# second-state/qwen3_asr_rs

Hardware: AMD Instinct MI355X
Metric: audio-seconds/sec (RTFx) Qwen3-ASR-0.6B greedy, 30s clips (higher is better)
Workload: dtype bf16; 1 GPU; Qwen3-ASR-0.6b bf16, batch=1 x 30s synthetic 16kHz clip per GPU, 100 new tokens (fixed, EOS ignored); clips_per_gpu=1, parallelism=dp1 (independent utterances per GPU, no data-path collective)

## Files before the change

qwen3_asr_rs_amd/csrc/engine.cpp:

```cpp
#include <hip/hip_runtime.h>

#include <sched.h>

#include <chrono>
#include <cmath>
#include <cstdio>
#include <cstring>
#include <map>
#include <memory>
#include <mutex>
#include <thread>

#include "engine_internal.h"

using namespace q3a;

namespace {

thread_local std::string g_last_error;

constexpr int kGemvMaxSeq = 2;

template <typename T>
void upload(DevBuf& b, const std::vector<T>& v, hipStream_t s) {
  b.ensure(std::max<size_t>(v.size() * sizeof(T), 16));
  if (!v.empty()) HIPCHK(hipMemcpyAsync(b.p, v.data(), v.size() * sizeof(T), hipMemcpyHostToDevice, s));
}

struct ProfEvent {
  int kclass;
  double bytes;
  hipEvent_t a, b;
};

template <class Build>
std::pair<std::vector<int32_t>, std::vector<int32_t>> concat_prompts(int B, Build&& build) {
  std::vector<int32_t> ids, lens(B);
  for (int s = 0; s < B; ++s) {
    lens[s] = build(s, nullptr);
    const size_t o = ids.size();
    ids.resize(o + lens[s]);
    build(s, ids.data() + o);
  }
  return {std::move(ids), std::move(lens)};
}

void require_utterance_ptrs(const char* what, const float* const* ptrs, int B) {
  for (int u = 0; u < B; ++u)
    if (!ptrs[u]) fail(std::string(what) + ": null utterance pointer");
}

}

namespace q3a {
struct KnobEntry { const char* key; const char* env; std::atomic<int> Knobs::*field; };
static const KnobEntry kKnobTable[] = {
    {"gemm256_min_tiles", "Q3A_GEMM256_MIN_TILES", &Knobs::gemm256_min_tiles},
    {"gemm256_persist", "Q3A_GEMM256_PERSIST", &Knobs::gemm256_persist},
    {"gemm256_group_m", "Q3A_GEMM256_GROUP_M", &Knobs::gemm256_group_m},
    {"dattn_batched_min_wgs", "Q3A_DATTN_BATCHED_MIN_WGS", &Knobs::dattn_batched_min_wgs},
    {"decode_group_size", "Q3A_DECODE_GROUP", &Knobs::decode_group_size},
    {"decode_parallel_groups", "Q3A_DECODE_PARALLEL", &Knobs::decode_parallel_groups},
    {"fuse_qkrope", "Q3A_FUSE_QKROPE", &Knobs::fuse_qkrope},
    {"skinny_q", "Q3A_SKINNY_Q", &Knobs::skinny_q},
    {"eos_run_ahead", "Q3A_EOS_RUN_AHEAD", &Knobs::eos_run_ahead},
    {"skinny_glu_hp3", "Q3A_SKINNY_GLU_HP3", &Knobs::skinny_glu_hp3},
    {"lm_head_prune", "Q3A_LM_HEAD_PRUNE", &Knobs::lm_head_prune},
    {"layer_taps", "Q3A_DEBUG_LAYER_TAPS", &Knobs::layer_taps},
    {"poison_attn_partials", nullptr, &Knobs::poison_attn_partials},
};
Knobs& knobs() {
  static Knobs k;
  static std::once_flag once;
  std::call_once(once, [] {
    for (const KnobEntry& t : kKnobTable)
      if (const char* e = t.env ? getenv(t.env) : nullptr) (k.*t.field).store(atoi(e));
  });
  return k;
}
}

namespace {

struct Taps {
  std::map<std::string, DevBuf> bufs;  std::map<std::string, size_t> bytes;
  DevBuf& reserve(const char* name, size_t n) { DevBuf& t = bufs[name]; t.ensure(n); bytes[name] = n; return t; }
  static bool light(const char* name) { return strcmp(name, "dec_last_hidden") == 0 || strcmp(name, "head_in") == 0; }
  void copy(int level, hipStream_t s, const char* name, const void* ptr, size_t n) {
    if (!level || n == 0 || (level == 2 && !light(name))) return;
    HIPCHK(hipMemcpyAsync(reserve(name, n).p, ptr, n, hipMemcpyDeviceToDevice, s));
  }
};

struct StepView {
  const Dims& d; const ArenaLayout& L; const q3a_opts& opts;
  uint8_t* const& arena; const uint32_t& arena_flags; const hipStream_t& stream;
  const std::vector<hipStream_t>& chain_streams;
  const std::vector<hipEvent_t>& join_ev; const hipEvent_t& fork_ev; const int& n_cu; int* const& host_prog_dev;
  std::vector<ProfEvent>* const& prof; Taps& taps;
  const int8_t* const& lm_q; const float* const& lm_qs; const int& lm_q_cols;
  const int &B, &max_ctx, &max_new, &gsize, &live_nsplit_, &attn_nsplit, &min_P_, &part_stride, &beam_w_;
  const size_t& kv_layer_elems; const bool& head_logits_;
  const int &k_parallel_groups, &k_skinny_q, &k_dattn_batched_min_wgs, &k_skinny_glu_hp3, &k_lm_head_prune;
  const bool& logit_bias_on_;
  const bool& sampling_on_;
  const bool& repetition_on_;

  bool precise() const { return opts.precise != 0; }
  bool token_lp() const { return opts.token_logprobs != 0; }
  bool kv_f32() const { return opts.precise != 0; }
  size_t kv_elem() const { return kv_f32() ? 4 : 2; }
  int fast_math() const { return precise() ? 0 : 1; }
  template <typename T> const T* w(uint64_t off) const { return reinterpret_cast<const T*>(arena + off); }
  const float* wf(uint64_t off) const { return w<float>(off); }
  const uint16_t* wh(uint64_t off) const { return w<uint16_t>(off); }
};

struct DecodeStep : StepView {
  DevBuf kcache, vcache, x_dec, d_pos, next_tok, out_ids, step_count, done, s_ln, s_qkv, s_ctx, s_act, logits, part_val, part_idx;
  DevBuf part_sum, out_lp;
  DevBuf blk_lo, blk_hi;
  DevBuf prune_stats;
  DevBuf attn_pm, attn_pl, attn_po, nn_x, nn_ss;
  DevBuf rope_cur, rope_cos, rope_sin;
  DevBuf n_done, forced_tok;
  DevBuf beam_cand_val, beam_cand_idx, beam_part_max, beam_part_sum, beam_topk_ids, beam_topk_lp, beam_score, beam_finished, beam_parent, beam_token;
  DevBuf beam_feed, beam_hist_parent, beam_hist_token, beam_hist_lp, beam_state, beam_lo;
  DevBuf logit_bias;
  DevBuf samp_params, samp_max, samp_sum;
  DevBuf rep_params;
  DevBuf draft_accepted;
  template <class Self, class F> static void each_buf(Self& s, F&& f) {
    for (auto* b : {&s.kcache, &s.vcache, &s.x_dec, &s.d_pos, &s.next_tok, &s.out_ids, &s.step_count, &s.done, &s.s_ln, &s.s_qkv, &s.s_ctx, &s.s_act, &s.logits,
                    &s.part_val, &s.part_idx, &s.part_sum, &s.out_lp, &s.blk_lo, &s.blk_hi, &s.prune_stats, &s.attn_pm, &s.attn_pl, &s.attn_po, &s.nn_x, &s.nn_ss,
                    &s.rope_cur, &s.rope_cos, &s.rope_sin, &s.n_done, &s.forced_tok,
                    &s.beam_cand_val, &s.beam_cand_idx, &s.beam_part_max, &s.beam_part_sum, &s.beam_topk_ids, &s.beam_topk_lp, &s.beam_score, &s.beam_finished,
                    &s.beam_parent, &s.beam_token, &s.beam_feed, &s.beam_hist_parent, &s.beam_hist_token, &s.beam_hist_lp, &s.beam_state, &s.beam_lo,
                    &s.logit_bias, &s.samp_params, &s.samp_max, &s.samp_sum, &s.rep_params, &s.draft_accepted})
      f(*b);
  }

  void tap(const char* name, const void* ptr, size_t bytes) { taps.copy(opts.debug_taps, stream, name, ptr, bytes); }
  template <class F> void timed(int kclass, double bytes, F&& fn) {
    if (!prof) return fn();
    ProfEvent pe{kclass, bytes, nullptr, nullptr};
    HIPCHK(hipEventCreate(&pe.a));
    HIPCHK(hipEventCreate(&pe.b));
    HIPCHK(hipEventRecord(pe.a, stream));
    fn();
    HIPCHK(hipEventRecord(pe.b, stream));
    prof->push_back(pe);
  }

  void* kc_layer(int l) { return (uint8_t*)kcache.p + (size_t)l * kv_layer_elems * kv_elem(); }
  void* vc_layer(int l) { return (uint8_t*)vcache.p + (size_t)l * kv_layer_elems * kv_elem(); }

  LmHeadPruneArgs prune_args(const GemvArgs& g) {
    LmHeadPruneArgs pa{};
    pa.g = g; pa.Wq = lm_q; pa.qcols = lm_q_cols; pa.qs = lm_qs;
    pa.blk_lo = blk_lo.as<float>(); pa.blk_hi = blk_hi.as<float>(); pa.stats = prune_stats.as<int>();
    pa.logit_bias = g.bias != nullptr;
    return pa;
  }

  const float* head_bias() const { return logit_bias_on_ ? logit_bias.as<float>() : nullptr; }

  void run_head(int advance) {
    const int S = B, H = d.hidden, V = d.vocab;
    const float* const hb = head_bias();
    const bool sample = sampling_on_, repeat = repetition_on_, store = head_logits_ || sample || repeat;
    tap("head_in", x_dec.p, (size_t)S * H * 4);
    const double wbytes = 2.0 * V * H;
    int n_part = 0;
    const ArgmaxPartials part{part_val.as<float>(), part_idx.as<int>(), token_lp() ? part_sum.as<float>() : nullptr, part_stride};
    if (S <= kGemvMaxSeq) {
      GemvArgs g{};
      g.fast_math = fast_math();
      g.x = x_dec.as<float>(); g.ldx = H; g.rms_w = wf(L.final_norm); g.eps = d.rms_eps;
      g.W = wh(L.lm_head); g.N = V; g.K = H; g.mode = 3; g.out = logits.as<float>(); g.ldo = V;
      g.part = part; g.bias = hb;
      LmHeadPruneArgs pa{};
      const bool prunable = S == 1 && !precise() && lm_q_cols > 0 && (pa = prune_args(g), !lm_head_prune_check(pa));
      if (prunable && opts.debug_taps == 1) {
        DevBuf& t = taps.reserve("lm_head_bound", (size_t)V * 8);
        LmHeadPruneArgs pd = pa;
        pd.dbg = t.as<float>(); pd.stats = nullptr;
        KCHK(launch_lm_head_approx(pd, stream));
      }
      if (prunable && k_lm_head_prune && !store) {
        g.out = nullptr; pa.g.out = nullptr;
        n_part = lm_head_rescore_groups(g, n_cu);
        timed(Q3A_KC_GEMV_LM_HEAD, (double)V * lm_q_cols, [&] { KCHK(launch_lm_head_approx(pa, stream)); });
        timed(Q3A_KC_ARGMAX, 0, [&] { KCHK(launch_lm_head_rescore(pa, n_part, stream)); });
      } else {
        n_part = gemv_blocks(g);
        timed(Q3A_KC_GEMV_LM_HEAD, wbytes, [&] { KCHK(launch_gemv(g, S, stream)); });
      }
    } else if (!precise()) {
      timed(Q3A_KC_NORM, 0, [&] { KCHK(launch_rmsnorm(x_dec.as<float>(), wf(L.final_norm), s_ln.as<float>(), S, H, d.rms_eps, stream, s_ln.as<uint16_t>())); });
      GemmEpilogue ep; ep.out = logits.as<float>(); ep.ldo = V; ep.bias = hb;
      if (S <= 32 && V % 4 == 0 && H % 64 == 0 && part_stride >= (V + 63) / 64) {
        ep.part = part;
        if (!store) ep.out = nullptr;
        n_part = (V + 63) / 64;
        timed(Q3A_KC_GEMM, wbytes, [&] { KCHK(launch_gemm16(s_ln.as<uint16_t>(), H, wh(L.lm_head), S, V, H, ep, false, stream)); });
      } else {
        timed(Q3A_KC_GEMM, wbytes, [&] { KCHK(launch_gemm16(s_ln.as<uint16_t>(), H, wh(L.lm_head), S, V, H, ep, false, stream)); });
        n_part = 128;
        if (!repeat) timed(Q3A_KC_ARGMAX, 0, [&] { KCHK(launch_argmax_partials(logits.as<float>(), V, S, part, n_part, stream)); });
      }
    } else {
      timed(Q3A_KC_NORM, 0, [&] { KCHK(launch_rmsnorm(x_dec.as<float>(), wf(L.final_norm), s_ln.as<float>(), S, H, d.rms_eps, stream)); });
      timed(Q3A_KC_GEMM, wbytes, [&] { batched_proj(s_ln.as<float>(), H, wh(L.lm_head), V, H, hb, 0, logits.as<float>(), V, nullptr); });
      n_part = 128;
      if (!repeat) timed(Q3A_KC_ARGMAX, 0, [&] { KCHK(launch_argmax_partials(logits.as<float>(), V, S, part, n_part, stream)); });
    }
    if (repeat) n_part = enqueue_repetition(part, !sample);
    FinalizeArgs f{};
    f.part = part; f.n_part = n_part; f.V = V; f.advance = advance; f.c = commit();
    if (sample) enqueue_sampler(f);
    timed(Q3A_KC_ARGMAX, 0, [&] { KCHK(launch_argmax_finalize(f, S, stream)); });
    if (sample && token_lp()) enqueue_sample_logprob();
  }
  StepCommit commit() const {
    StepCommit c{};
    c.next_tok = next_tok.as<int>(); c.out_ids = out_ids.as<int>(); c.out_stride = max_new; c.out_lp = token_lp() ? out_lp.as<float>() : nullptr;
    c.step_count = step_count.as<int>(); c.pos = d_pos.as<int>();
    c.done = done.as<uint8_t>(); c.n_done = n_done.as<int>(); c.n_seq = B; c.host_progress = host_prog_dev;
    c.embed = wh(L.embed); c.H = d.hidden; c.x_next = x_dec.as<float>(); c.eos0 = kEos0; c.eos1 = kEos1;
    c.cos_t = rope_cos.as<float>(); c.sin_t = rope_sin.as<float>(); c.rope_cur = rope_cur.as<float>();
    c.nn = first_layer_norm_out();
    return c;
  }
  void enqueue_draft_accept(DraftAcceptArgs a) {
    a.n_seq = B; a.accepted = draft_accepted.as<int>(); a.c = commit();
    timed(Q3A_KC_ARGMAX, 0, [&] { KCHK(launch_draft_accept(a, stream)); });
  }
  void enqueue_set_tokens(const int* tok) { KCHK(launch_set_tokens(tok, B, commit(), stream)); }
  void enqueue_forced_tokens(const int32_t* ids) {
    HIPCHK(hipMemcpy(forced_tok.p, ids, (size_t)B * 4, hipMemcpyHostToDevice));
    enqueue_set_tokens(forced_tok.as<int>());
  }
  int enqueue_repetition(const ArgmaxPartials& part, bool partials) {
    RepeatArgs ra{};
    ra.logits = logits.as<float>(); ra.S = B; ra.V = d.vocab; ra.params = rep_params.as<uint32_t>();
    ra.out_ids = out_ids.as<int>(); ra.out_stride = max_new; ra.step_count = step_count.as<int>();
    timed(Q3A_KC_ARGMAX, 0, [&] { KCHK(launch_repeat_apply(ra, stream)); });
    constexpr int kRepeatParts = 128;
    if (partials) timed(Q3A_KC_ARGMAX, 0, [&] { KCHK(launch_argmax_partials(ra.logits, ra.V, ra.S, part, kRepeatParts, stream)); });
    return kRepeatParts;
  }
  void enqueue_sampler(FinalizeArgs& f) {
    SampleArgs sa{};
    sa.logits = logits.as<float>(); sa.S = B; sa.V = d.vocab; sa.params = samp_params.as<uint32_t>(); sa.step_count = step_count.as<int>();
    sa.chunk_max = samp_max.as<float>(); sa.chunk_sum = samp_sum.as<float>();
    f.part.sum = nullptr; f.c.out_lp = nullptr; f.n_part = sample_chunks(d.vocab);
    sa.part = f.part;
    timed(Q3A_KC_ARGMAX, 0, [&] { KCHK(launch_sample(sa, stream)); });
  }
  void enqueue_sample_logprob() {
    SampleLogprobArgs sl{};
    sl.logits = logits.as<float>(); sl.S = B; sl.V = d.vocab; sl.chunk_max = samp_max.as<float>(); sl.chunk_sum = samp_sum.as<float>();
    sl.next_tok = next_tok.as<int>(); sl.step_count = step_count.as<int>(); sl.out_lp = out_lp.as<float>(); sl.out_stride = max_new;
    timed(Q3A_KC_ARGMAX, 0, [&] { KCHK(launch_sample_logprob(sl, stream)); });
  }

  bool prenorm_path() const { return B > kGemvMaxSeq && !precise(); }
  bool skinny_q() const {
    auto whole = [](int K) { const int st = K / 32, per = (st + 7) / 8, unr = per <= 2 ? 2 : per <= 4 ? 4 : per <= 8 ? 8 : 12; return K % 256 == 0 && per % unr == 0; };
    return k_skinny_q != 0 && !precise() && d.hidden % 64 == 0 && whole(d.q_dim()) && whole(d.inter);
  }
  int nn_parts() const { return d.hidden / (skinny_q() ? 8 : 16); }
  int n_groups(int b) const { return b <= kGemvMaxSeq ? 1 : (b + gsize - 1) / gsize; }
  size_t nn_x_stride() const { return (size_t)32 * d.hidden; }
  size_t nn_ss_stride() const { return (size_t)nn_parts() * 32; }
  uint16_t* nn_x_g(int g) const { return nn_x.as<uint16_t>() + (size_t)g * nn_x_stride(); }
  float* nn_ss_g(int g) const { return nn_ss.as<float>() + (size_t)g * nn_ss_stride(); }
  float* s_ctx_g(int g) const { return s_ctx.as<float>() + (size_t)g * 32 * d.q_dim(); }
  float* s_act_g(int g) const { return s_act.as<float>() + (size_t)g * 32 * d.inter; }
  NextNormOut first_layer_norm_out() const {
    NextNormOut nn{};
    if (prenorm_path()) {
      nn.next_w = wf(L.dec[0].in_ln); nn.next_xw16f = nn_x.as<uint16_t>(); nn.next_ss = nn_ss.as<float>(); nn.nparts = nn_parts();
      nn.group_stride_x = (long)nn_x_stride(); nn.group_stride_ss = (long)nn_ss_stride(); nn.group_size = gsize;
    }
    return nn;
  }

  void batched_proj(const float* x, int ldx, const uint16_t* W, int N, int K, const float* bias, int mode, float* out,
                    int ldo, const float* resid) {
    const int S = B;
    if (S <= 32) {
      SkinnyArgs sk{};
      sk.fast_math = fast_math();
      sk.x = x; sk.ldx = ldx; sk.S = S; sk.W = W; sk.N = N; sk.K = K; sk.bias = bias; sk.mode = mode; sk.out = out; sk.ldo = ldo; sk.resid = resid;
      KCHK(launch_skinny(sk, precise(), stream));
    } else {
      GemmEpilogue ep; ep.out = out; ep.ldo = ldo; ep.bias = bias; ep.resid = (mode == 1) ? resid : nullptr;
      KCHK(launch_gemm(x, ldx, W, S, N, K, ep, mode == 2, precise(), stream));
    }
  }

  struct Proj {
    const uint16_t* W;
    int N, K;
    const float* bias;
    int mode;
    int kclass;
    double bytes;
  };
  struct LayerProjs { Proj qkv, o, gu, down; };
  LayerProjs layer_projs(int li) const {
    const DecLayerOff& l = L.dec[li];
    const int H = d.hidden, I = d.inter, QD = d.q_dim(), QKV = d.qkv_dim();
    auto proj = [&](uint64_t w_off, int N, int K, uint32_t bias_flag, uint64_t b_off, int mode, int kclass) {
      return Proj{wh(w_off), N, K, (arena_flags & bias_flag) ? wf(b_off) : nullptr, mode, kclass, 2.0 * N * K};
    };
    return {proj(l.qkv_w, QKV, H, kFlagDecQkvBias, l.qkv_b, 0, Q3A_KC_GEMV), proj(l.o_w, H, QD, kFlagDecOBias, l.o_b, 1, Q3A_KC_GEMV_O),
            proj(l.gu_w, 2 * I, H, kFlagDecMlpBias, l.gu_b, 2, Q3A_KC_GEMV), proj(l.down_w, H, I, kFlagDecMlpBias, l.down_b, 1, Q3A_KC_GEMV_DOWN)};
  }
  template <class Args> Args proj_args(const Proj& p) const {
    Args a{};
    a.fast_math = fast_math(); a.eps = d.rms_eps;
    a.W = p.W; a.N = p.N; a.K = p.K; a.ldx = p.K; a.bias = p.bias; a.mode = p.mode; a.ldo = p.mode == 2 ? p.N / 2 : p.N;
    return a;
  }
  GemvArgs gemv_args(const Proj& p) const { return proj_args<GemvArgs>(p); }
  SkinnyArgs skinny_args(const Proj& p, int S) const { SkinnyArgs k = proj_args<SkinnyArgs>(p); k.S = S; return k; }

  void decode_layer(int li, int grp, int s0, int S, hipStream_t ks) {
    const int H = d.hidden, QKV = d.qkv_dim();
    const bool gemv = B <= kGemvMaxSeq;
    const DecLayerOff& l = L.dec[li];
    const LayerProjs pj = layer_projs(li);
    float* const x = x_dec.as<float>() + (size_t)s0 * H;
    float* const qkv = s_qkv.as<float>() + (size_t)s0 * QKV;
    const size_t kv_seq = (size_t)d.n_kv * max_ctx * 128 * kv_elem();
    DecodeAttnArgs da{};
    da.qkv = qkv; da.pos = d_pos.as<int>() + s0; da.eps = d.rms_eps;
    da.rope_cur = rope_cur.as<float>() + (size_t)s0 * 128;
    da.pm = attn_pm.as<float>() + (size_t)s0 * d.n_q * attn_nsplit; da.pl = attn_pl.as<float>() + (size_t)s0 * d.n_q * attn_nsplit;
    da.po = attn_po.as<float>() + (size_t)s0 * d.n_q * attn_nsplit * 128; da.nsplit = live_nsplit_;
    da.n_q = d.n_q; da.n_kv = d.n_kv; da.max_ctx = max_ctx; da.scale_div = sqrtf((float)d.head_dim);
    da.q_norm = wf(l.q_norm); da.k_norm = wf(l.k_norm);
    da.kcache = (uint8_t*)kc_layer(li) + (size_t)s0 * kv_seq; da.vcache = (uint8_t*)vc_layer(li) + (size_t)s0 * kv_seq;
    if (gemv) {
      auto run = [&](const Proj& p, const GemvArgs& a) { timed(p.kclass, p.bytes, [&] { KCHK(launch_gemv(a, S, ks)); }); };
      GemvArgs g = gemv_args(pj.qkv);
      g.x = x; g.rms_w = wf(l.in_ln); g.out = qkv;
      run(pj.qkv, g);
      timed(Q3A_KC_DECODE_ATTN, 0, [&] { KCHK(launch_decode_attn(da, S, kv_f32(), ks)); });
      GemvArgs o = gemv_args(pj.o);
      if (std::min(S, 4) * d.n_q * live_nsplit_ <= GEMV_ATTN_MAX_TABLE) {
        o.attn_pm = da.pm; o.attn_pl = da.pl; o.attn_po = da.po;
        o.attn_nsplit = live_nsplit_; o.attn_heads = d.n_q; o.attn_fast_exp = fast_math();
      } else {
        timed(Q3A_KC_DECODE_ATTN, 0, [&] { KCHK(launch_attn_combine(da.pm, da.pl, da.po, live_nsplit_, S, d.n_q, s_ctx_g(grp), ks)); });
        o.x = s_ctx_g(grp);
      }
      o.out = x; o.resid = x;
      run(pj.o, o);
      GemvArgs u = gemv_args(pj.gu);
      u.x = x; u.rms_w = wf(l.post_ln); u.out = s_act_g(grp);
      run(pj.gu, u);
      GemvArgs dn = gemv_args(pj.down);
      dn.x = s_act_g(grp); dn.out = x; dn.resid = x;
      run(pj.down, dn);
      return;
    }
    const bool b16 = !precise(), pre = prenorm_path();
    uint16_t* const s_ctx16 = b16 ? reinterpret_cast<uint16_t*>(s_ctx_g(grp)) : nullptr;
    uint16_t* const s_act16 = b16 ? reinterpret_cast<uint16_t*>(s_act_g(grp)) : nullptr;
    auto run = [&](const Proj& p, const SkinnyArgs& a) { timed(Q3A_KC_GEMM, p.bytes, [&] { KCHK(launch_skinny(a, precise(), ks)); }); };
    auto from_residual = [&](SkinnyArgs& a, const float* norm_w) {
      a.x = x;
      if (pre) { a.xw16f = nn_x_g(grp); a.ss_parts = nn_ss_g(grp); a.ss_nparts = nn_parts(); }
      else a.rms_w = norm_w;
    };
    auto to_residual = [&](SkinnyArgs& a, const float* next_w) {
      a.out = x; a.resid = x;
      a.qsplit = b16 && skinny_q();
      if (pre && next_w) { a.next_w = next_w; a.next_xw16f = nn_x_g(grp); a.next_ss = nn_ss_g(grp); }
    };
    SkinnyArgs q = skinny_args(pj.qkv, S);
    from_residual(q, wf(l.in_ln));
    q.out = qkv;
    run(pj.qkv, q);
    if (S * d.n_kv >= k_dattn_batched_min_wgs) {
      if (b16) { da.out16 = s_ctx16; da.out_frag = 1; } else da.out = s_ctx_g(grp);
      da.trim_prologue = min_P_ < 2 * 128;
      timed(Q3A_KC_DECODE_ATTN, 0, [&] { KCHK(launch_decode_attn_batched(da, S, kv_f32(), ks)); });
    } else {
      timed(Q3A_KC_DECODE_ATTN, 0, [&] { KCHK(launch_decode_attn(da, S, kv_f32(), ks)); });
      timed(Q3A_KC_DECODE_ATTN, 0, [&] { KCHK(launch_attn_combine(da.pm, da.pl, da.po, live_nsplit_, S, d.n_q, s_ctx_g(grp), ks, s_ctx16, b16)); });
    }
    SkinnyArgs o = skinny_args(pj.o, S);
    o.x = s_ctx_g(grp); o.x16 = s_ctx16; o.x16_frag = b16;
    to_residual(o, wf(l.post_ln));
    run(pj.o, o);
    SkinnyArgs u = skinny_args(pj.gu, S);
    from_residual(u, wf(l.post_ln));
    u.out = s_act_g(grp); u.out16 = s_act16; u.out16_frag = b16;
    u.n_cu = n_cu;
    u.glu_hp3 = k_skinny_glu_hp3;
    run(pj.gu, u);
    SkinnyArgs dn = skinny_args(pj.down, S);
    dn.x = s_act_g(grp); dn.x16 = s_act16; dn.x16_frag = b16;
    to_residual(dn, li + 1 < d.dec_layers ? wf(L.dec[li + 1].in_ln) : nullptr);
    run(pj.down, dn);
  }

  bool forks() const { return n_groups(B) > 1 && !prof && k_parallel_groups != 0; }
  void enqueue_decode_step() {
    const int ng = n_groups(B);
    const bool chains = forks();
    if (chains) HIPCHK(hipEventRecord(fork_ev, stream));
    for (int g = 0; g < ng; ++g) {
      const int s0 = ng == 1 ? 0 : g * gsize;
      const int S = ng == 1 ? B : std::min(gsize, B - s0);
      hipStream_t ks = (chains && g > 0) ? chain_streams[g - 1] : stream;
      if (chains && g > 0) HIPCHK(hipStreamWaitEvent(ks, fork_ev, 0));
      for (int li = 0; li < d.dec_layers; ++li) decode_layer(li, g, s0, S, ks);
      if (chains && g > 0) {
        HIPCHK(hipEventRecord(join_ev[g - 1], ks));
        HIPCHK(hipStreamWaitEvent(stream, join_ev[g - 1], 0));
      }
    }
    run_head(1);
  }

  bool uses_key_splits() const {
    if (B <= kGemvMaxSeq) return true;
    const int ng = n_groups(B);
    const int smallest = ng == 1 ? B : std::min(gsize, B - (ng - 1) * gsize);
    return smallest * d.n_kv < k_dattn_batched_min_wgs;
  }

  void enqueue_step() {
    enqueue_decode_step();
    if (beam_w_ > 0) enqueue_beam_round();
  }
  void enqueue_beam_round() {
    const int W = beam_w_, S = B, U = B / W;
    BeamTopkArgs t{};
    t.logits = logits.as<float>(); t.S = S; t.V = d.vocab; t.W = W;
    t.cand_val = beam_cand_val.as<float>(); t.cand_idx = beam_cand_idx.as<int>();
    t.part_max = beam_part_max.as<float>(); t.part_sum = beam_part_sum.as<float>();
    t.out_ids = beam_topk_ids.as<int>(); t.out_lp = beam_topk_lp.as<float>();
    timed(Q3A_KC_ARGMAX, 0, [&] { KCHK(launch_beam_topk(t, stream)); });
    BeamAdvanceArgs a{};
    a.U = U; a.W = W; a.topk_ids = t.out_ids; a.topk_lp = t.out_lp;
    a.score = beam_score.as<float>(); a.finished = beam_finished.as<uint8_t>();
    a.parent = beam_parent.as<int>(); a.token = beam_token.as<int>(); a.feed = beam_feed.as<int>();
    a.hist_parent = beam_hist_parent.as<int>(); a.hist_token = beam_hist_token.as<int>(); a.hist_lp = beam_hist_lp.as<float>();
    a.hist_cap = max_new; a.state = beam_state.as<int>();
    a.pos = d_pos.as<int>(); a.lo = beam_lo.as<int>(); a.hi_bias = -1;
    a.host_progress = host_prog_dev + 2; a.eos0 = kEos0; a.eos1 = kEos1;
    timed(Q3A_KC_ARGMAX, 0, [&] { KCHK(launch_beam_advance(a, stream)); });
    KvReorderArgs r{};
    r.kcache = kcache.p; r.vcache = vcache.p; r.elem_bytes = (int)kv_elem(); r.layers = d.dec_layers; r.S = S; r.n_kv = d.n_kv; r.max_ctx = max_ctx;
    r.parent = a.parent; r.lo = a.lo; r.hi = a.pos; r.hi_bias = -1; r.all_done = a.state + BEAM_ST_ALL_DONE;
    timed(Q3A_KC_OTHER, 0, [&] { KCHK(launch_kv_reorder(r, stream)); });
    timed(Q3A_KC_OTHER, 0, [&] { enqueue_set_tokens(a.feed); });
  }
};

}

struct q3a_engine {
  Dims d;
  ArenaLayout L;
  q3a_opts opts{};
  int device = 0;
  hipStream_t stream = nullptr;
  uint8_t* arena = nullptr;
  bool own_arena = false;
  uint32_t arena_flags = 0;
  std::string err;

  DevBuf dft, filt_t, pos_emb;
  int rope_positions = 0;

  int B = 0;
  std::vector<int64_t> n_samples, pcm_off, mel_off;
  std::vector<int> n_frames, n_chunks, T, tok_off;
  int total_chunks = 0, total_T = 0, max_frames = 0;
  bool have_mel = false, have_enc = false, have_prefill = false;
  std::vector<int> P, seq_off;
  int total_P = 0, max_ctx = 0, max_new = 0;
  std::vector<AttnSeg> enc_segs_h;
  int enc_max_seg = 0;

  DevBuf pcm, d_pcm_off, d_n_samples, d_mel_off, d_n_frames, mel, gmax, d_chunk_utt, d_chunk_frame0;
  DevBuf conv1, conv2, conv3, conv3_rowmap, convout_rowmap;
  DevBuf enc_x, enc_ln, enc_qkv, enc_ctx, enc_ffn, enc_segs, audio_embeds;
  DevBuf ids, audio_rowmap, row_seq, row_pos, dec_segs, last_rows;
  DevBuf dec_x, dec_ln, dec_qkv, dec_ctx, dec_act;
  DevBuf lm_q_buf, lm_qs_buf;
  const int8_t* lm_q = nullptr; const float* lm_qs = nullptr;
  int lm_q_cols = 0;
  DevBuf enc_ctx16, dec_ctx16;
  DevBuf dec_q16;
  int n_cu = 256;
  int* host_prog = nullptr;
  int* host_prog_dev = nullptr;
  DevBuf zero_page;
  int part_stride = 0, attn_nsplit = 0;
  size_t kv_layer_elems = 0;

  int gsize = 32;
  int k_parallel_groups = 1, k_skinny_q = 1, k_dattn_batched_min_wgs = 128, k_skinny_glu_hp3 = 1, k_lm_head_prune = 1;
  std::vector<hipStream_t> chain_streams;
  std::vector<hipEvent_t> join_ev;
  hipEvent_t fork_ev = nullptr;

  static constexpr size_t kGraphCacheMax = 16;
  std::vector<std::pair<std::string, hipGraphExec_t>> graph_cache;
  int pos_hi_ = 0, live_nsplit_ = 0;
  int min_P_ = 0;

  hipStream_t up_stream = nullptr;
  void* pin_p = nullptr;
  size_t pin_cap = 0;
  std::vector<hipEvent_t> up_ev;
  hipEvent_t up_t0 = nullptr, up_t1 = nullptr;
  q3a_io_timings io{};
  bool geom_valid = false;

  q3a_timings timings{};
  hipEvent_t ev[5] = {nullptr, nullptr, nullptr, nullptr, nullptr};
  std::vector<ProfEvent>* prof = nullptr;
  Taps taps;

  bool fixed_mode_ = false;
  bool head_logits_ = true;
  int beam_w_ = 0;
  bool logit_bias_on_ = false;
  int logit_bias_finite_ = 0;
  bool sampling_on_ = false;
  uint32_t samp_words_[4] = {0, 0, 0, 0};
  bool logit_bias_eos_open_ = true;
  bool repetition_on_ = false;
  float rep_penalty_ = 1.f;
  int rep_ngram_ = 0;

  DecodeStep step{StepView{d, L, opts, arena, arena_flags, stream, chain_streams, join_ev, fork_ev, n_cu, host_prog_dev, prof, taps, lm_q, lm_qs, lm_q_cols,
                           B, max_ctx, max_new, gsize, live_nsplit_, attn_nsplit, min_P_, part_stride, beam_w_, kv_layer_elems, head_logits_,
                           k_parallel_groups, k_skinny_q, k_dattn_batched_min_wgs, k_skinny_glu_hp3, k_lm_head_prune, logit_bias_on_, sampling_on_, repetition_on_}};

  bool precise() const { return step.precise(); }
  bool token_lp() const { return step.token_lp(); }
  bool kv_f32() const { return step.kv_f32(); }
  size_t kv_elem() const { return step.kv_elem(); }
  size_t act_elem() const { return precise() ? 4 : 2; }
  bool valu_attn() const { return precise() || opts.valu_attention; }
  const float* wf(uint64_t off) const { return step.wf(off); }
  const uint16_t* wh(uint64_t off) const { return step.wh(off); }

  void tap(const char* name, const void* ptr, size_t bytes) { step.tap(name, ptr, bytes); }
  void tap_act(const char* name, const void* ptr, size_t elems) {
    if (!opts.debug_taps || elems == 0 || opts.debug_taps == 2) return;
    if (precise()) return tap(name, ptr, elems * 4);
    KCHK(launch_from_bf16((const uint16_t*)ptr, taps.reserve(name, elems * 4).as<float>(), elems, stream));
  }

  void act_gemm(const DevBuf& x, int lda, const uint16_t* W, int M, int N, int K, const GemmEpilogue& ep, bool glu) {
    if (precise()) KCHK(launch_gemm(x.as<float>(), lda, W, M, N, K, ep, glu, true, stream));
    else KCHK(launch_gemm16(x.as<uint16_t>(), lda, W, M, N, K, ep, glu, stream));
  }
  void act_conv(const DevBuf& x, int imgs, int H, int Wd, int C, const uint16_t* W, int Cout, const GemmEpilogue& ep) {
    if (precise()) KCHK(launch_conv3x3s2_gemm(x.as<float>(), imgs, H, Wd, C, W, Cout, ep, true, stream));
    else KCHK(launch_conv3x3s2_gemm16(x.as<uint16_t>(), zero_page.as<uint16_t>(), imgs, H, Wd, C, W, Cout, ep, stream));
  }
  void act_out(GemmEpilogue& ep, const DevBuf& buf) const {
    if (precise()) ep.out = buf.as<float>(); else ep.out16 = buf.as<uint16_t>();
  }
  uint16_t* act16(const DevBuf& buf) const { return precise() ? nullptr : buf.as<uint16_t>(); }

  float stage_ms(int i, int j) { float ms = 0.f; HIPCHK(hipEventElapsedTime(&ms, ev[i], ev[j])); return ms; }

  void init_common(const std::string& model_dir, int dev, const q3a_opts* o) {
    if (o) opts = *o; else q3a_opts_default(&opts);
    if (opts.max_new_tokens <= 0) opts.max_new_tokens = 4096;
    d = parse_config_file(model_dir + "/config.json");
    validate_dims(d);
    L = plan_arena(d);
    device = dev;
    int n_dev = 0;
    hipError_t e = hipGetDeviceCount(&n_dev);
    if (e != hipSuccess || n_dev == 0)
      fail("no HIP device available: libq3asr_hip has no CPU fallback (hipGetDeviceCount: " + std::string(hipGetErrorString(e)) + ")");
    if (dev < 0 || dev >= n_dev) fail("device index out of range");
    HIPCHK(hipSetDevice(dev));
    KCHK(skinny_init());
    (void)hipDeviceGetAttribute(&n_cu, hipDeviceAttributeMultiprocessorCount, dev);
    HIPCHK(hipStreamCreateWithFlags(&stream, hipStreamNonBlocking));
    for (auto& x : ev) HIPCHK(hipEventCreate(&x));
    HIPCHK(hipHostMalloc((void**)&host_prog, 64, hipHostMallocMapped));
    memset(host_prog, 0, 64);
    HIPCHK(hipHostGetDevicePointer((void**)&host_prog_dev, host_prog, 0));
    step.n_done.ensure(64);
    step.prune_stats.ensure(8);
    HIPCHK(hipMemsetAsync(step.prune_stats.p, 0, 8, stream));
    if (!d.aligner()) {
      step.logit_bias.ensure((size_t)d.vocab * 4);
      HIPCHK(hipMemsetAsync(step.logit_bias.p, 0, (size_t)d.vocab * 4, stream));
      logit_bias_finite_ = d.vocab;
      step.samp_params.ensure(16);
      step.rep_params.ensure(16);
    }
  }

  void init_tables() {
    auto dftm = make_dft_matrix(400, 416);
    auto filt = make_mel_filterbank_T(d.n_mels, 400, 16000, 202);
    auto pe = make_sinusoid_rows(d.tokens_per_chunk(), d.enc_d);
    upload(dft, dftm, stream);
    upload(filt_t, filt, stream);
    upload(pos_emb, pe, stream);
    zero_page.ensure(256);
    HIPCHK(hipMemsetAsync(zero_page.p, 0, 256, stream));
    ensure_rope(8192);
    HIPCHK(hipStreamSynchronize(stream));
  }

  void ensure_rope(int n_pos) {
    if (n_pos <= rope_positions) return;
    int n = std::max(n_pos, 8192);
    std::vector<float> c, s;
    make_rope_tables(n, d.head_dim, d.rope_theta, c, s);
    HIPCHK(hipStreamSynchronize(stream));
    upload(step.rope_cos, c, stream);
    upload(step.rope_sin, s, stream);
    HIPCHK(hipStreamSynchronize(stream));
    rope_positions = n;
  }

  void init_lm_head_q() {
    const int cols = lm_head_q_cols(d.hidden);
    if (precise() || d.aligner() || cols == 0 || d.hidden % 8 != 0) return;
    lm_q_buf.ensure((size_t)d.vocab * cols);
    lm_qs_buf.ensure((size_t)d.vocab * 16);
    KCHK(launch_lm_head_quantize(wh(L.lm_head), d.vocab, d.hidden, lm_q_buf.as<int8_t>(), lm_qs_buf.as<float>(), stream));
    HIPCHK(hipStreamSynchronize(stream));
    lm_q = lm_q_buf.as<int8_t>(); lm_qs = lm_qs_buf.as<float>(); lm_q_cols = cols;
  }

  void check_arena_header() {
    ArenaHeader h;
    HIPCHK(hipMemcpy(&h, arena, sizeof(h), hipMemcpyDeviceToHost));
    if (h.magic != kArenaMagic || h.version != kArenaVersion) fail("weight arena: bad magic/version");
    if (h.total_bytes != L.total) fail("weight arena: size does not match config.json");
    arena_flags = h.flags;
  }

  void set_batch(const int64_t* ns, int b) {
    have_mel = have_enc = have_prefill = false;
    if (b <= 0) { B = 0; fail("batch must be >= 1"); }
    if (geom_valid && b == B && (int)n_samples.size() == b && std::equal(ns, ns + b, n_samples.begin())) return;
    geom_valid = false;
    B = 0;
    for (int u = 0; u < b; ++u)
      if (ns[u] < 161) fail("utterance too short: reflection padding needs more than 160 samples (src/mel.rs:63-65)");
    n_samples.assign(ns, ns + b);
    pcm_off.resize(b); mel_off.resize(b); n_frames.resize(b); n_chunks.resize(b); T.resize(b); tok_off.resize(b);
    std::vector<int> chunk_utt, chunk_frame0, convout_map, conv3_map;
    enc_segs_h.clear();
    int64_t po = 0, mo = 0;
    int tok = 0;
    total_chunks = 0; max_frames = 0; enc_max_seg = 0;
    const int cf = d.chunk_frames(), tpc = d.tokens_per_chunk(), cpw = d.chunks_per_window();
    for (int u = 0; u < b; ++u) {
      pcm_off[u] = po;
      po += (ns[u] + 3) & ~int64_t(3);
      int F = (int)((ns[u] + 159) / 160);
      n_frames[u] = F;
      max_frames = std::max(max_frames, F);
      mel_off[u] = mo;
      mo += (int64_t)F * d.n_mels;
      int nc = (F + cf - 1) / cf;
      n_chunks[u] = nc;
      tok_off[u] = tok;
      std::vector<int> valid(nc);
      for (int c = 0; c < nc; ++c) {
        int frames = std::min(cf, F - c * cf);
        valid[c] = Dims::feat_len(frames);
        chunk_utt.push_back(u);
        chunk_frame0.push_back(c * cf);
        for (int t = 0; t < tpc; ++t) convout_map.push_back(t < valid[c] ? tok + t : -1);
        tok += valid[c];
      }
      T[u] = tok - tok_off[u];
      int t0 = tok_off[u];
      if (nc <= cpw) {
        enc_segs_h.push_back(AttnSeg{t0, T[u], (int64_t)t0 * 3 * d.enc_d});
        enc_max_seg = std::max(enc_max_seg, T[u]);
      } else {
        for (int c0 = 0; c0 < nc; c0 += cpw) {
          int len = 0;
          for (int c = c0; c < std::min(nc, c0 + cpw); ++c) len += valid[c];
          enc_segs_h.push_back(AttnSeg{t0, len, (int64_t)t0 * 3 * d.enc_d});
          enc_max_seg = std::max(enc_max_seg, len);
          t0 += len;
        }
      }
      total_chunks += nc;
    }
    total_T = tok;
    const int f3 = d.freq3();
    conv3_map.resize((size_t)total_chunks * f3 * tpc);
    for (int c = 0; c < total_chunks; ++c)
      for (int f = 0; f < f3; ++f)
        for (int t = 0; t < tpc; ++t) conv3_map[((size_t)c * f3 + f) * tpc + t] = (c * tpc + t) * f3 + f;
    pcm.ensure((size_t)po * 4);
    upload(d_pcm_off, pcm_off, stream);
    upload(d_n_samples, n_samples, stream);
    upload(d_mel_off, mel_off, stream);
    upload(d_n_frames, n_frames, stream);
    upload(d_chunk_utt, chunk_utt, stream);
    upload(d_chunk_frame0, chunk_frame0, stream);
    upload(convout_rowmap, convout_map, stream);
    upload(conv3_rowmap, conv3_map, stream);
    upload(enc_segs, enc_segs_h, stream);
    mel.ensure((size_t)mo * 4);
    gmax.ensure((size_t)b * 4);
    HIPCHK(hipStreamSynchronize(stream));
    B = b;
    geom_valid = true;
  }

  void upload_pcm(const float* host, const int64_t* ns, int b) {
    set_batch(ns, b);
    int64_t src = 0;
    for (int u = 0; u < b; ++u) {
      HIPCHK(hipMemcpyAsync(pcm.as<float>() + pcm_off[u], host + src, (size_t)ns[u] * 4, hipMemcpyHostToDevice, stream));
      src += ns[u];
    }
    HIPCHK(hipStreamSynchronize(stream));
  }

  void upload_ptrs_and_mel(const float* const* ptrs, const int64_t* ns, int b) {
    const auto w0 = std::chrono::steady_clock::now();
    set_batch(ns, b);
    static const int mode = [] { const char* e = getenv("Q3A_UPLOAD_MODE"); return e ? atoi(e) : 1; }();
    static const int thr_env = [] { const char* e = getenv("Q3A_UPLOAD_THREADS"); return e ? atoi(e) : -1; }();
    static const int pieces_env = [] { const char* e = getenv("Q3A_UPLOAD_PIECES"); return e ? atoi(e) : 8; }();
    io = q3a_io_timings{};
    io.mode = mode;
    HIPCHK(hipEventRecord(ev[0], stream));
    const size_t total = (size_t)(pcm_off[b - 1] + ((ns[b - 1] + 3) & ~int64_t(3))) * 4;
    bool staged = mode != 0;
    if (staged && total > pin_cap) {
      if (up_stream) HIPCHK(hipStreamSynchronize(up_stream));
      if (pin_p) (void)hipHostFree(pin_p);
      pin_p = nullptr; pin_cap = 0;
      const size_t want = (total + (size_t(1) << 20) - 1) & ~((size_t(1) << 20) - 1);
      if (hipHostMalloc(&pin_p, want, hipHostMallocDefault) == hipSuccess && pin_p) pin_cap = want;
      else { (void)hipGetLastError(); pin_p = nullptr; staged = false; io.mode = 0; }
    }
    if (!staged) {
      for (int u = 0; u < b; ++u)
        HIPCHK(hipMemcpyAsync(pcm.as<float>() + pcm_off[u], ptrs[u], (size_t)ns[u] * 4, hipMemcpyHostToDevice, stream));
      HIPCHK(hipStreamSynchronize(stream));
      io.pieces = b;
      run_mel();
      HIPCHK(hipEventRecord(ev[1], stream));
      io.stage_ms = std::chrono::duration<float, std::milli>(std::chrono::steady_clock::now() - w0).count();
      return;
    }
    if (!up_stream) {
      HIPCHK(hipStreamCreateWithFlags(&up_stream, hipStreamNonBlocking));
      HIPCHK(hipEventCreate(&up_t0));
      HIPCHK(hipEventCreate(&up_t1));
    }
    HIPCHK(hipStreamSynchronize(up_stream));
    const int want_pieces = std::max(1, std::min(b, pieces_env));
    std::vector<int> first;
    {
      const size_t per = (total + want_pieces - 1) / want_pieces;
      size_t acc = 0;
      first.push_back(0);
      for (int u = 0; u < b; ++u) {
        acc += (size_t)ns[u] * 4;
        if (acc >= per && u + 1 < b && (int)first.size() < want_pieces) { first.push_back(u + 1); acc = 0; }
      }
      first.push_back(b);
    }
    const int np = (int)first.size() - 1;
    while ((int)up_ev.size() < np) {
      hipEvent_t e2;
      HIPCHK(hipEventCreateWithFlags(&e2, hipEventDisableTiming));
      up_ev.push_back(e2);
    }
    const int nthr = thr_env >= 0 ? std::min(thr_env, np) : (total >= (size_t(8) << 20) ? std::min(8, np) : 0);
    io.pieces = np;
    io.threads = nthr;
    std::vector<std::atomic<int>> ready(np);
    for (auto& r : ready) r.store(0, std::memory_order_relaxed);
    std::atomic<int> next{0};
    uint8_t* const pin = (uint8_t*)pin_p;
    auto copy_piece = [&](int p) {
      for (int u = first[p]; u < first[p + 1]; ++u) memcpy(pin + (size_t)pcm_off[u] * 4, ptrs[u], (size_t)ns[u] * 4);
      ready[p].store(1, std::memory_order_release);
    };
    struct Joiner {
      std::vector<std::thread> th;
      ~Joiner() { for (auto& t : th) if (t.joinable()) t.join(); }
    } workers;
    for (int t = 0; t < nthr; ++t)
      workers.th.emplace_back([&] { for (int p; (p = next.fetch_add(1, std::memory_order_relaxed)) < np;) copy_piece(p); });
    MelBatch mb{pcm.as<float>(), d_pcm_off.as<int64_t>(), d_n_samples.as<int64_t>(), d_mel_off.as<int64_t>(),
                d_n_frames.as<int>(), mel.as<float>(), gmax.as<unsigned>()};
    HIPCHK(hipEventRecord(up_t0, up_stream));
    for (int p = 0; p < np; ++p) {
      if (nthr == 0) copy_piece(p);
      for (unsigned spins = 0; !ready[p].load(std::memory_order_acquire);)
        if (++spins > 256) sched_yield();
      const int u0 = first[p], u1 = first[p + 1];
      const size_t o0 = (size_t)pcm_off[u0] * 4, o1 = (size_t)(pcm_off[u1 - 1] + ns[u1 - 1]) * 4;
      HIPCHK(hipMemcpyAsync((uint8_t*)pcm.p + o0, pin + o0, o1 - o0, hipMemcpyHostToDevice, up_stream));
      HIPCHK(hipEventRecord(up_ev[p], up_stream));
      HIPCHK(hipStreamWaitEvent(stream, up_ev[p], 0));
      MelBatch piece = mb;
      piece.pcm_off += u0; piece.n_samples += u0; piece.mel_off += u0; piece.n_frames += u0; piece.gmax_key += u0;
      int mf = 0;
      for (int u = u0; u < u1; ++u) mf = std::max(mf, n_frames[u]);
      KCHK(launch_mel(piece, u1 - u0, mf, dft.as<float>(), filt_t.as<float>(), stream));
    }
    HIPCHK(hipEventRecord(up_t1, up_stream));
    io.stage_ms = std::chrono::duration<float, std::milli>(std::chrono::steady_clock::now() - w0).count();
    mel_done();
    HIPCHK(hipEventRecord(ev[1], stream));
  }

  void run_mel() {
    MelBatch mb{pcm.as<float>(), d_pcm_off.as<int64_t>(), d_n_samples.as<int64_t>(), d_mel_off.as<int64_t>(),
                d_n_frames.as<int>(), mel.as<float>(), gmax.as<unsigned>()};
    KCHK(launch_mel(mb, B, max_frames, dft.as<float>(), filt_t.as<float>(), stream));
    mel_done();
  }
  void mel_done() {
    have_mel = true;
    size_t bytes = 0;
    for (int u = 0; u < B; ++u) bytes += (size_t)n_frames[u] * d.n_mels * 4;
    tap("mel", mel.p, bytes);
  }

  void run_encoder() {
    if (!have_mel) fail("q3a_encode: no mel (call q3a_mel first)");
    const int C = d.conv_ch, D = d.enc_d, Fn = d.enc_ffn;
    const int H1 = Dims::conv_len(d.n_mels), W1 = Dims::conv_len(d.chunk_frames());
    const int H2 = Dims::conv_len(H1), W2 = Dims::conv_len(W1);
    const int H3 = Dims::conv_len(H2), W3 = Dims::conv_len(W2);
    const bool sp = precise();
    const size_t nch = (size_t)total_chunks;
    const size_t ae = act_elem();
    conv1.ensure(nch * H1 * W1 * C * ae);
    conv2.ensure(nch * H2 * W2 * C * ae);
    conv3.ensure(nch * H3 * W3 * C * ae);
    const size_t Tt = (size_t)total_T;
    const bool qkv16 = !valu_attn();
    enc_x.ensure(Tt * D * 4); enc_ln.ensure(Tt * D * ae); enc_qkv.ensure(Tt * 3 * D * (qkv16 ? 2 : 4));
    enc_ctx.ensure(Tt * D * (valu_attn() ? 4 : ae));
    if (valu_attn() && !sp) enc_ctx16.ensure(Tt * D * 2);
    enc_ffn.ensure(Tt * Fn * ae); audio_embeds.ensure(Tt * d.enc_out * 4);

    ChunkTable ct{d_chunk_utt.as<int>(), d_chunk_frame0.as<int>()};
    KCHK(launch_conv1(mel.as<float>(), d_mel_off.as<int64_t>(), d_n_frames.as<int>(), ct, total_chunks, d.n_mels,
                      d.chunk_frames(), wf(L.conv1_w), wf(L.conv1_b), C, conv1.as<float>(), stream, act16(conv1)));
    tap_act("conv1", conv1.p, nch * H1 * W1 * C);
    {
      GemmEpilogue ep;
      act_out(ep, conv2); ep.ldo = C; ep.bias = wf(L.conv2_b); ep.act = 1;
      act_conv(conv1, total_chunks, H1, W1, C, wh(L.conv2_w), C, ep);
      tap_act("conv2", conv2.p, nch * H2 * W2 * C);
    }
    {
      GemmEpilogue ep;
      act_out(ep, conv3); ep.ldo = C; ep.bias = wf(L.conv3_b); ep.act = 1; ep.rowmap = conv3_rowmap.as<int>();
      act_conv(conv2, total_chunks, H2, W2, C, wh(L.conv3_w), C, ep);
      tap_act("conv3", conv3.p, nch * H3 * W3 * C);
    }
    {
      GemmEpilogue ep;
      ep.out = enc_x.as<float>(); ep.ldo = D;
      ep.bias = (arena_flags & kFlagConvOutBias) ? wf(L.conv_out_b) : nullptr;
      ep.rowmap = convout_rowmap.as<int>();
      ep.addend = pos_emb.as<float>(); ep.addend_period = W3;
      act_gemm(conv3, H3 * C, wh(L.conv_out_w), total_chunks * W3, D, H3 * C, ep, false);
      tap("enc_in", enc_x.p, Tt * D * 4);
    }
    AttnArgs at{};
    at.q = enc_qkv.as<float>(); at.q_rs = 3 * D;
    at.k = enc_qkv.as<float>() + D; at.v = enc_qkv.as<float>() + 2 * D; at.kv_hs = 64; at.kv_rs = 3 * D;
    if (qkv16) {
      at.q16 = enc_qkv.as<uint16_t>();
      at.k = enc_qkv.as<uint16_t>() + D; at.v = enc_qkv.as<uint16_t>() + 2 * D;
    }
    at.o = enc_ctx.as<float>(); at.o_rs = D;
    at.o16 = valu_attn() ? nullptr : enc_ctx.as<uint16_t>();
    at.segs = enc_segs.as<AttnSeg>(); at.n_segs = (int)enc_segs_h.size(); at.max_len = enc_max_seg;
    at.n_kv_heads = d.enc_heads; at.scale_div = 8.0f;
    const DevBuf& ctx_in = (valu_attn() && !sp) ? enc_ctx16 : enc_ctx;
    for (int li = 0; li < d.enc_layers; ++li) {
      const EncLayerOff& e = L.enc[li];
      KCHK(launch_layernorm(enc_x.as<float>(), wf(e.ln1_w), wf(e.ln1_b), enc_ln.as<float>(), total_T, D, 1e-5f, stream, act16(enc_ln)));
      {
        GemmEpilogue ep; ep.ldo = 3 * D; ep.bias = wf(e.qkv_b);
        if (qkv16) ep.out16 = enc_qkv.as<uint16_t>(); else ep.out = enc_qkv.as<float>();
        act_gemm(enc_ln, D, wh(e.qkv_w), total_T, 3 * D, D, ep, false);
      }
      if (valu_attn()) {
        KCHK(launch_attn_enc(at, stream));
        if (!sp) KCHK(launch_to_bf16(enc_ctx.as<float>(), enc_ctx16.as<uint16_t>(), Tt * D, stream));
      } else {
        KCHK(launch_fattn_enc(at, stream));
      }
      {
        GemmEpilogue ep; ep.out = enc_x.as<float>(); ep.ldo = D; ep.bias = wf(e.out_b); ep.resid = enc_x.as<float>();
        act_gemm(ctx_in, D, wh(e.out_w), total_T, D, D, ep, false);
      }
      KCHK(launch_layernorm(enc_x.as<float>(), wf(e.ln2_w), wf(e.ln2_b), enc_ln.as<float>(), total_T, D, 1e-5f, stream, act16(enc_ln)));
      {
        GemmEpilogue ep; act_out(ep, enc_ffn); ep.ldo = Fn; ep.bias = wf(e.fc1_b); ep.act = 1;
        act_gemm(enc_ln, D, wh(e.fc1_w), total_T, Fn, D, ep, false);
      }
      {
        GemmEpilogue ep; ep.out = enc_x.as<float>(); ep.ldo = D; ep.bias = wf(e.fc2_b); ep.resid = enc_x.as<float>();
        act_gemm(enc_ffn, Fn, wh(e.fc2_w), total_T, D, Fn, ep, false);
      }
      if (li == 0) tap("enc_layer0", enc_x.p, Tt * D * 4);
      if (opts.debug_taps == 1 && knobs().layer_taps.load() != 0) {
        char name[32];
        snprintf(name, sizeof(name), "E%02d_x", li);
        tap(name, enc_x.p, Tt * D * 4);
      }
    }
    tap("enc_last", enc_x.p, Tt * D * 4);
    KCHK(launch_layernorm(enc_x.as<float>(), wf(L.ln_post_w), wf(L.ln_post_b), enc_ln.as<float>(), total_T, D, 1e-5f, stream, act16(enc_ln)));
    {
      GemmEpilogue ep; act_out(ep, enc_ffn); ep.ldo = D; ep.bias = wf(L.proj1_b); ep.act = 1;
      act_gemm(enc_ln, D, wh(L.proj1_w), total_T, D, D, ep, false);
    }
    {
      GemmEpilogue ep; ep.out = audio_embeds.as<float>(); ep.ldo = d.enc_out; ep.bias = wf(L.proj2_b);
      act_gemm(enc_ffn, D, wh(L.proj2_w), total_T, d.enc_out, D, ep, false);
    }
    tap("audio_embeds", audio_embeds.p, Tt * d.enc_out * 4);
    HIPCHK(hipGetLastError());
    have_enc = true;
  }

  void setup_prompts(const int32_t* ids_h, const int32_t* lens, int b, int max_new_req, bool before_encoder = false) {
    if (!have_enc && !before_encoder) fail("q3a_prefill: no encoder output (call q3a_encode first)");
    if (b != B) fail("q3a_prefill: batch size differs from the encoded batch");
    P.assign(lens, lens + b);
    beam_w_ = 0;
    seq_off.resize(b);
    std::vector<int> rowseq, rowpos, amap((size_t)total_T, -1), last(b);
    int off = 0, maxP = 0;
    for (int s = 0; s < b; ++s) {
      seq_off[s] = off;
      int na = 0;
      for (int i = 0; i < P[s]; ++i) {
        rowseq.push_back(s);
        rowpos.push_back(i);
        int id = ids_h[off + i];
        if (id < 0 || id >= d.vocab) fail("q3a_prefill: token id out of range");
        if (id == kAudioPad) {
          if (na >= T[s]) fail("q3a_prefill: more <|audio_pad|> tokens than encoder tokens");
          amap[(size_t)tok_off[s] + na] = off + i;
          ++na;
        }
      }
      if (na != T[s]) fail("q3a_prefill: number of <|audio_pad|> tokens does not match the encoder output length");
      if (P[s] <= 0) fail("q3a_prefill: empty prompt");
      last[s] = off + P[s] - 1;
      off += P[s];
      maxP = std::max(maxP, P[s]);
    }
    total_P = off;
    max_new = std::min(std::max(max_new_req, 1), opts.max_new_tokens);
    max_ctx = ((maxP + max_new + 1 + 127) / 128) * 128;
    pos_hi_ = maxP;
    min_P_ = *std::min_element(P.begin(), P.end());
    {
      static const int pad = [] { const char* e = getenv("Q3A_CTX_PAD"); return e ? atoi(e) : 0; }();
      if (pad > 0) max_ctx += (pad + 127) / 128 * 128;
    }
    ensure_rope(max_ctx + 1);
    std::vector<int> ids_v(ids_h, ids_h + total_P);
    std::vector<AttnSeg> segs(b);
    for (int s = 0; s < b; ++s)
      segs[s] = AttnSeg{seq_off[s], P[s], (int64_t)s * d.n_kv * max_ctx * 128};
    upload(ids, ids_v, stream);
    upload(row_seq, rowseq, stream);
    upload(row_pos, rowpos, stream);
    upload(audio_rowmap, amap, stream);
    upload(last_rows, last, stream);
    upload(dec_segs, segs, stream);
    upload(step.d_pos, P, stream);
    const size_t Pt = (size_t)total_P, H = d.hidden;
    dec_x.ensure(Pt * H * 4); dec_ln.ensure(Pt * H * act_elem()); dec_qkv.ensure(Pt * d.qkv_dim() * 4);
    dec_ctx.ensure(Pt * d.q_dim() * (valu_attn() ? 4 : act_elem())); dec_act.ensure(Pt * d.inter * act_elem());
    if (!valu_attn()) dec_q16.ensure(Pt * d.q_dim() * 2);
    if (valu_attn() && !precise()) dec_ctx16.ensure(Pt * d.q_dim() * 2);
    kv_layer_elems = (size_t)b * d.n_kv * max_ctx * 128;
    step.kcache.ensure(kv_layer_elems * d.dec_layers * kv_elem());
    step.vcache.ensure(kv_layer_elems * d.dec_layers * kv_elem());
    step.rope_cur.ensure((size_t)b * 128 * 4);
    {
      Knobs& kn = knobs();
      const int gs = kn.decode_group_size.load();
      gsize = (gs >= 1 && gs <= 32) ? gs : 32;
      k_parallel_groups = kn.decode_parallel_groups.load(); k_skinny_q = kn.skinny_q.load();
      k_dattn_batched_min_wgs = kn.dattn_batched_min_wgs.load();
      k_skinny_glu_hp3 = kn.skinny_glu_hp3.load();
      k_lm_head_prune = kn.lm_head_prune.load();
    }
    const size_t ng = (size_t)step.n_groups(b);
    step.nn_x.ensure(ng * 32 * H * 2); step.nn_ss.ensure((size_t)ng * (H / 8) * 32 * 4);
    step.x_dec.ensure((size_t)b * H * 4); step.next_tok.ensure((size_t)b * 4); step.forced_tok.ensure((size_t)b * 4); step.draft_accepted.ensure((size_t)b * 8);
    step.out_ids.ensure((size_t)b * max_new * 4); step.step_count.ensure((size_t)b * 4); step.done.ensure((size_t)b);
    step.s_ln.ensure((size_t)b * H * 4); step.s_qkv.ensure((size_t)b * d.qkv_dim() * 4); step.s_ctx.ensure(ng * 32 * d.q_dim() * 4);
    step.s_act.ensure(ng * 32 * d.inter * 4); step.logits.ensure((size_t)b * d.vocab * 4);
    part_stride = std::max(128, (d.vocab + 3) / 4);
    step.part_val.ensure((size_t)b * part_stride * 4); step.part_idx.ensure((size_t)b * part_stride * 4);
    if (token_lp()) { step.part_sum.ensure((size_t)b * part_stride * 4); step.out_lp.ensure((size_t)b * max_new * 4); }
    if (sampling_on_) { step.samp_max.ensure((size_t)b * sample_chunks(d.vocab) * 4); step.samp_sum.ensure((size_t)b * sample_chunks(d.vocab) * 4); }
    {
      const size_t nblk4 = ((size_t)(d.vocab + 15) / 16 + 3) & ~size_t(3);
      step.blk_lo.ensure(nblk4 * 4); step.blk_hi.ensure(nblk4 * 4);
    }
    attn_nsplit = (max_ctx + dattn_keys_per_split(kv_f32()) - 1) / dattn_keys_per_split(kv_f32());
    {
      const size_t n_stat = (size_t)b * d.n_q * attn_nsplit;
      step.attn_pm.ensure((n_stat + 8) * 4); step.attn_pl.ensure((n_stat + 8) * 4);
      step.attn_po.ensure(n_stat * 128 * 4);
      if (knobs().poison_attn_partials.load() != 0) {
        HIPCHK(hipMemsetAsync(step.attn_pm.p, 0xFF, step.attn_pm.cap, stream));
        HIPCHK(hipMemsetAsync(step.attn_pl.p, 0xFF, step.attn_pl.cap, stream));
        HIPCHK(hipMemsetAsync(step.attn_po.p, 0xFF, step.attn_po.cap, stream));
      }
    }
    HIPCHK(hipMemsetAsync(step.step_count.p, 0, (size_t)b * 4, stream));
    HIPCHK(hipMemsetAsync(step.done.p, 0, (size_t)b, stream));
    HIPCHK(hipMemsetAsync(step.n_done.p, 0, 64, stream));
    HIPCHK(hipMemsetAsync(step.out_ids.p, 0, (size_t)b * max_new * 4, stream));
    if (token_lp()) HIPCHK(hipMemsetAsync(step.out_lp.p, 0, (size_t)b * max_new * 4, stream));
    HIPCHK(hipStreamSynchronize(stream));
    for (auto cs : chain_streams) HIPCHK(hipStreamSynchronize(cs));
    __atomic_store_n(&host_prog[0], 0, __ATOMIC_RELAXED);
    __atomic_store_n(&host_prog[1], 0, __ATOMIC_RELAXED);
    drain_retired_graphs();
    {
      bool any = false;
      DecodeStep::each_buf(step, [&](DevBuf& sb) { any = any || sb.grew; sb.grew = false; });
      if (any) drop_graphs();
    }
  }

  void run_prefill() {
    run_prefill_layers();
    const int H = d.hidden;
    KCHK(launch_gather_rows(dec_x.as<float>(), last_rows.as<int>(), B, H, step.x_dec.as<float>(), stream));
    tap("dec_last_hidden", step.x_dec.p, (size_t)B * H * 4);
    step.run_head(0);
    tap("logits", step.logits.p, (size_t)B * d.vocab * 4);
    HIPCHK(hipGetLastError());
    have_prefill = true;
  }

  void run_prefill_layers() {
    const int H = d.hidden, I = d.inter, QD = d.q_dim(), QKV = d.qkv_dim();
    const bool sp = precise();
    KCHK(launch_embed(ids.as<int>(), total_P, wh(L.embed), H, kAudioPad, dec_x.as<float>(), stream));
    KCHK(launch_scatter_rows(audio_embeds.as<float>(), audio_rowmap.as<int>(), total_T, d.hidden, dec_x.as<float>(), stream));
    tap("dec_embed", dec_x.p, (size_t)total_P * H * 4);
    AttnArgs at{};
    at.q = dec_qkv.as<float>(); at.q_rs = QKV; at.kv_hs = (int64_t)max_ctx * 128; at.kv_rs = 128;
    at.o = dec_ctx.as<float>(); at.o_rs = QD; at.segs = dec_segs.as<AttnSeg>(); at.n_segs = B;
    at.max_len = *std::max_element(P.begin(), P.end()); at.n_kv_heads = d.n_kv;
    at.scale_div = sqrtf((float)d.head_dim);
    at.o16 = valu_attn() ? nullptr : dec_ctx.as<uint16_t>();
    if (!valu_attn()) { at.q16 = dec_q16.as<uint16_t>(); at.q_rs = QD; }
    const DevBuf& ctx_in = (valu_attn() && !sp) ? dec_ctx16 : dec_ctx;
    const bool qkv_bias = arena_flags & kFlagDecQkvBias, o_bias = arena_flags & kFlagDecOBias, mlp_bias = arena_flags & kFlagDecMlpBias;
    const bool fuse_rope = knobs().fuse_qkrope.load() != 0 && !valu_attn() && !precise() && d.head_dim == 128 && gemm256_eligible(total_P, QKV, H) && H % 64 == 0;
    const bool layer_taps = opts.debug_taps && knobs().layer_taps.load() != 0;
    for (int li = 0; li < d.dec_layers; ++li) {
      const DecLayerOff& l = L.dec[li];
      auto ltap = [&](const char* what, const void* ptr, size_t bytes) {
        if (!layer_taps) return;
        char name[32];
        snprintf(name, sizeof(name), "L%02d_%s", li, what);
        tap(name, ptr, bytes);
      };
      KCHK(launch_rmsnorm(dec_x.as<float>(), wf(l.in_ln), dec_ln.as<float>(), total_P, H, d.rms_eps, stream, act16(dec_ln)));
      ltap("ln1", dec_ln.p, (size_t)total_P * H * act_elem());
      RopeKvArgs rk{};
      rk.qkv = dec_qkv.as<float>(); rk.row_seq = row_seq.as<int>(); rk.row_pos = row_pos.as<int>();
      rk.q_norm = wf(l.q_norm); rk.k_norm = wf(l.k_norm); rk.eps = d.rms_eps;
      rk.cos_t = step.rope_cos.as<float>(); rk.sin_t = step.rope_sin.as<float>();
      rk.kcache = step.kc_layer(li); rk.vcache = step.vc_layer(li); rk.n_q = d.n_q; rk.n_kv = d.n_kv; rk.max_ctx = max_ctx;
      rk.q16 = valu_attn() ? nullptr : dec_q16.as<uint16_t>();
      if (fuse_rope) {
        KCHK(launch_gemm256_qkrope(dec_ln.as<uint16_t>(), H, wh(l.qkv_w), total_P, H, qkv_bias ? wf(l.qkv_b) : nullptr, rk, stream));
      } else {
        GemmEpilogue ep; ep.out = dec_qkv.as<float>(); ep.ldo = QKV; ep.bias = qkv_bias ? wf(l.qkv_b) : nullptr;
        act_gemm(dec_ln, H, wh(l.qkv_w), total_P, QKV, H, ep, false);
        KCHK(launch_qknorm_rope_kv(rk, total_P, kv_f32(), stream));
      }
      at.k = step.kc_layer(li); at.v = step.vc_layer(li);
      if (fuse_rope) {
        ltap("qkvs", dec_qkv.p, std::min((size_t)1024, (size_t)total_P) * QKV * 4);
      }
      if (!valu_attn()) ltap("q", dec_q16.p, (size_t)total_P * QD * 2);
      ltap("k", step.kc_layer(li), (size_t)B * d.n_kv * max_ctx * 128 * kv_elem());
      ltap("v", step.vc_layer(li), (size_t)B * d.n_kv * max_ctx * 128 * kv_elem());
      if (valu_attn()) {
        KCHK(launch_attn_prefill(at, d.n_q / d.n_kv, kv_f32(), stream));
        if (!sp) KCHK(launch_to_bf16(dec_ctx.as<float>(), dec_ctx16.as<uint16_t>(), (size_t)total_P * QD, stream));
      } else {
        KCHK(launch_fattn_prefill(at, d.n_q / d.n_kv, stream));
      }
      ltap("attn", ctx_in.p, (size_t)total_P * QD * act_elem());
      {
        GemmEpilogue ep; ep.out = dec_x.as<float>(); ep.ldo = H; ep.resid = dec_x.as<float>(); ep.bias = o_bias ? wf(l.o_b) : nullptr;
        act_gemm(ctx_in, QD, wh(l.o_w), total_P, H, QD, ep, false);
      }
      ltap("o", dec_x.p, (size_t)total_P * H * 4);
      KCHK(launch_rmsnorm(dec_x.as<float>(), wf(l.post_ln), dec_ln.as<float>(), total_P, H, d.rms_eps, stream, act16(dec_ln)));
      ltap("ln2", dec_ln.p, (size_t)total_P * H * act_elem());
      {
        GemmEpilogue ep; act_out(ep, dec_act); ep.ldo = I; ep.bias = mlp_bias ? wf(l.gu_b) : nullptr;
        act_gemm(dec_ln, H, wh(l.gu_w), total_P, 2 * I, H, ep, true);
      }
      ltap("act", dec_act.p, (size_t)total_P * I * act_elem());
      {
        GemmEpilogue ep; ep.out = dec_x.as<float>(); ep.ldo = H; ep.resid = dec_x.as<float>(); ep.bias = mlp_bias ? wf(l.down_b) : nullptr;
        act_gemm(dec_act, I, wh(l.down_w), total_P, H, I, ep, false);
      }
      ltap("x", dec_x.p, (size_t)total_P * H * 4);
      if (li == 0) tap("dec_layer0", dec_x.p, (size_t)total_P * H * 4);
    }
  }

  void require_asr(const char* what) const {
    if (d.aligner()) fail(std::string(what) + ": this engine holds a forced aligner (classify_num in config.json); use q3a_align*");
  }
  void require_aligner(const char* what) const {
    if (!d.aligner()) fail(std::string(what) + ": not a forced-aligner checkpoint (config.json has no thinker_config.classify_num)");
  }
  std::vector<int> align_marker_rows(const int32_t* ids_h, const int32_t* lens, int b, int stride, int32_t* counts) const {
    std::vector<int> rows;
    int off = 0;
    for (int s = 0; s < b; ++s) {
      int n = 0;
      for (int i = 0; i < lens[s]; ++i)
        if (ids_h[off + i] == d.timestamp_token_id) { rows.push_back(off + i); ++n; }
      if (n > stride)
        fail("q3a_align: utterance " + std::to_string(s) + " has " + std::to_string(n) + " timestamp markers, more than stride " + std::to_string(stride));
      counts[s] = n;
      off += lens[s];
    }
    return rows;
  }
  template <class Head>
  void run_prefill_then_head(const std::vector<int>& rows, float& head_ms, Head&& enqueue_head) {
    have_prefill = false;
    HIPCHK(hipEventRecord(ev[2], stream));
    run_prefill_layers();
    HIPCHK(hipEventRecord(ev[3], stream));
    if (!rows.empty()) {
      upload(align_rows, rows, stream);
      enqueue_head();
    }
    HIPCHK(hipEventRecord(ev[4], stream));
    HIPCHK(hipStreamSynchronize(stream));
    HIPCHK(hipGetLastError());
    timings.prefill_ms = stage_ms(2, 4);
    head_ms = stage_ms(3, 4);
    timings.decode_ms = 0.f; timings.decode_steps = 0; timings.batch = B; timings.total_audio_tokens = total_T;
    timings.total_prompt_tokens = total_P;
  }
  void decode_timings(int steps) {
    front_and_total_timings();
    timings.prefill_ms = stage_ms(2, 3);
    timings.decode_ms = stage_ms(3, 4);
    timings.decode_steps = steps; timings.batch = B; timings.total_audio_tokens = total_T; timings.total_prompt_tokens = total_P;
  }
  void front_and_total_timings() {
    timings.mel_ms = stage_ms(0, 1);
    timings.encoder_ms = stage_ms(1, 2);
    timings.total_ms = stage_ms(0, 4);
  }
  void fill_row_head(RowHeadArgs& a, int M, int N, bool log_sum, bool want_logits) {
    const int H = d.hidden, planes = precise() ? 2 : 1, n_part = align_head_parts(N);
    align_xn.ensure((size_t)planes * align_rows_padded(M) * H * 2);
    align_pval.ensure((size_t)M * n_part * 4); align_pidx.ensure((size_t)M * n_part * 4);
    if (log_sum) score_psum.ensure((size_t)M * n_part * 4);
    if (want_logits) align_logits.ensure((size_t)M * N * 4);
    a.x = dec_x.as<float>(); a.ldx = H; a.rows = align_rows.as<int>(); a.M = M;
    a.norm_w = wf(L.final_norm); a.eps = d.rms_eps; a.W = wh(L.lm_head); a.N = N; a.K = H;
    a.planes = planes; a.xn = align_xn.as<uint16_t>();
    a.part = ArgmaxPartials{align_pval.as<float>(), align_pidx.as<int>(), log_sum ? score_psum.as<float>() : nullptr, n_part};
    a.logits = want_logits ? align_logits.as<float>() : nullptr; a.ldl = (size_t)N;
  }
  ScoreHeadArgs score_head_args(int M, const std::vector<int>& targets, bool want_logits) {
    ScoreHeadArgs a{};
    fill_row_head(a, M, d.vocab, true, want_logits);
    upload(score_tgt, targets, stream);
    score_out.ensure((size_t)M * 4 * 4);
    a.targets = score_tgt.as<int>();
    a.tgt_logit = score_out.as<float>(); a.lp = score_out.as<float>() + M;
    a.top_id = score_out.as<int>() + 2 * (size_t)M; a.top_lp = score_out.as<float>() + 3 * (size_t)M;
    return a;
  }
  void run_align(const std::vector<int>& rows, const int32_t* counts, int stride, int32_t* out_classes, float* logits_out) {
    const int M = (int)rows.size(), N = d.classify_num;
    run_prefill_then_head(rows, align_head_ms, [&] {
      AlignHeadArgs a{};
      fill_row_head(a, M, N, false, logits_out != nullptr);
      align_cls.ensure((size_t)M * 4);
      a.classes = align_cls.as<int>();
      KCHK(launch_align_head(a, stream));
    });
    std::vector<int> cls((size_t)M);
    if (M > 0) HIPCHK(hipMemcpy(cls.data(), align_cls.p, (size_t)M * 4, hipMemcpyDeviceToHost));
    if (M > 0 && logits_out) HIPCHK(hipMemcpy(logits_out, align_logits.p, (size_t)M * N * 4, hipMemcpyDeviceToHost));
    for (int s = 0, k = 0; s < B; ++s)
      for (int i = 0; i < counts[s]; ++i) out_classes[(size_t)s * stride + i] = cls[k++];
  }
  DevBuf align_rows, align_xn, align_pval, align_pidx, align_cls, align_logits;
  float align_head_ms = 0.f;

  struct ScorePlan {
    std::vector<int32_t> ids, lens;
    std::vector<int> rows, targets;
  };
  void check_given_id(const char* what, const std::string& noun, int32_t y) const {
    if (y < 0 || y >= d.vocab) fail(std::string(what) + ": " + noun + " id " + std::to_string(y) + " out of range (vocabulary " + std::to_string(d.vocab) + ")");
    if (y == kAudioPad)
      fail(std::string(what) + ": <|audio_pad|> (" + std::to_string(kAudioPad) + ") cannot be a " + (noun == "target" ? noun : noun + " id") + ": the engine finds audio rows by this id");
  }
  ScorePlan score_plan(const char* what, const int32_t* prompt_ids, const int32_t* prompt_lens, const int32_t* target_ids,
                       const int32_t* target_lens, int b, int stride) const {
    ScorePlan sp;
    sp.lens.resize(b);
    size_t po = 0, to = 0;
    for (int s = 0; s < b; ++s) {
      const int p = prompt_lens[s], n = target_lens[s];
      if (p <= 0) fail(std::string(what) + ": empty prompt");
      if (n < 0 || (n > 0 && !target_ids)) fail(std::string(what) + ": bad target length");
      if (n > stride)
        fail(std::string(what) + ": utterance " + std::to_string(s) + " has " + std::to_string(n) + " targets, more than stride " + std::to_string(stride));
      const int row0 = (int)sp.ids.size() + p - 1;
      sp.ids.insert(sp.ids.end(), prompt_ids + po, prompt_ids + po + p);
      for (int i = 0; i < n; ++i) {
        const int32_t y = target_ids[to + i];
        check_given_id(what, "target", y);
        if (i + 1 < n) sp.ids.push_back(y);
        sp.rows.push_back(row0 + i);
        sp.targets.push_back(y);
      }
      sp.lens[s] = p + std::max(n - 1, 0);
      po += p; to += n;
    }
    return sp;
  }
  void run_score(const ScorePlan& sp, const int32_t* target_lens, int stride, float* out_lp, int32_t* out_top_ids, float* out_top_lp,
                 float* logits_out) {
    const int M = (int)sp.rows.size(), V = d.vocab;
    run_prefill_then_head(sp.rows, score_head_ms, [&] { KCHK(launch_score_head(score_head_args(M, sp.targets, logits_out != nullptr), stream)); });
    if (M == 0) return;
    std::vector<float> res((size_t)M * 4);
    HIPCHK(hipMemcpy(res.data(), score_out.p, res.size() * 4, hipMemcpyDeviceToHost));
    if (logits_out) HIPCHK(hipMemcpy(logits_out, align_logits.p, (size_t)M * V * 4, hipMemcpyDeviceToHost));
    const float* lp = res.data() + M;
    const int32_t* ti = reinterpret_cast<const int32_t*>(res.data()) + 2 * (size_t)M;
    const float* tl = res.data() + 3 * (size_t)M;
    for (int s = 0, k = 0; s < B; ++s)
      for (int i = 0; i < target_lens[s]; ++i, ++k) {
        out_lp[(size_t)s * stride + i] = lp[k];
        if (out_top_ids) out_top_ids[(size_t)s * stride + i] = ti[k];
        if (out_top_lp) out_top_lp[(size_t)s * stride + i] = tl[k];
      }
  }
  DevBuf score_tgt, score_psum, score_out;
  float score_head_ms = 0.f;

  struct DraftPlan {
    std::vector<int32_t> ids, lens;
    std::vector<int> rows, targets;
    std::vector<int> words;
    std::vector<int> plen, dlen;
  };
  void draft_check(const char* what) const {
    require_asr(what);
    if (sampling_on_) fail(std::string(what) + ": sampling is on (q3a_set_sampling with temperature > 0): a sampled id is not the argmax of its row -- turn it off first");
    if (repetition_on_) fail(std::string(what) + ": repetition control is on (q3a_set_repetition): its choice depends on the history, not on the row alone -- turn it off first");
    if (beam_w_ > 0) fail(std::string(what) + ": a beam search owns the decode state (a new q3a_prefill returns to the greedy step)");
  }
  DraftPlan draft_plan(const char* what, const int32_t* prompt_ids, const int32_t* prompt_lens, const int32_t* draft_ids, const int32_t* draft_lens,
                       int b, int max_new_eff) const {
    DraftPlan dp;
    dp.lens.resize(b); dp.plen.resize(b); dp.dlen.resize(b);
    dp.words.assign((size_t)2 * b + 1, 0);
    size_t po = 0, to = 0;
    for (int s = 0; s < b; ++s) {
      const int p = prompt_lens[s], n = draft_lens[s];
      if (p <= 0) fail(std::string(what) + ": empty prompt");
      if (n < 0 || (n > 0 && !draft_ids)) fail(std::string(what) + ": bad draft length");
      if (n > max_new_eff)
        fail(std::string(what) + ": utterance " + std::to_string(s) + " has a draft of " + std::to_string(n) + " ids, more than max_new " + std::to_string(max_new_eff));
      const int row0 = (int)dp.ids.size() + p - 1;
      dp.ids.insert(dp.ids.end(), prompt_ids + po, prompt_ids + po + p);
      for (int i = 0; i < n; ++i) {
        const int32_t y = draft_ids[to + i];
        check_given_id(what, "draft", y);
        if (y == kEos0 || y == kEos1) fail(std::string(what) + ": an EOS id (" + std::to_string(y) + ") cannot be a draft id: a draft ends where its ids end");
        dp.ids.push_back(y);
        dp.words.push_back(y);
        dp.rows.push_back(row0 + i);
        dp.targets.push_back(y);
      }
      dp.rows.push_back(row0 + n);
      dp.targets.push_back(0);
      dp.lens[s] = p + n; dp.plen[s] = p; dp.dlen[s] = n;
      dp.words[s + 1] = dp.words[s] + n;
      dp.words[(size_t)b + 1 + s] = p;
      po += p; to += n;
    }
    return dp;
  }
  void run_prefill_draft(const DraftPlan& dp, std::vector<int>& acc, float* logits_out) {
    const int M = (int)dp.rows.size(), V = d.vocab;
    have_prefill = false;
    run_prefill_layers();
    upload(align_rows, dp.rows, stream);
    upload(draft_in, dp.words, stream);
    ScoreHeadArgs a = score_head_args(M, dp.targets, logits_out != nullptr);
    a.bias = step.head_bias();
    KCHK(launch_score_head(a, stream));
    DraftAcceptArgs da{};
    da.draft_off = draft_in.as<int>(); da.prompt_len = da.draft_off + B + 1; da.draft = da.prompt_len + B;
    da.top_id = a.top_id; da.top_lp = a.top_lp;
    step.enqueue_draft_accept(da);
    HIPCHK(hipStreamSynchronize(stream));
    HIPCHK(hipGetLastError());
    acc.resize((size_t)2 * B);
    HIPCHK(hipMemcpy(acc.data(), step.draft_accepted.p, acc.size() * 4, hipMemcpyDeviceToHost));
    if (logits_out) HIPCHK(hipMemcpy(logits_out, align_logits.p, (size_t)M * V * 4, hipMemcpyDeviceToHost));
    pos_hi_ = 0; min_P_ = 0x7fffffff;
    for (int s = 0; s < B; ++s) {
      if (acc[s] < 0 || acc[s] > dp.dlen[s]) fail("draft accept: the device returned a first mismatch outside the draft");
      pos_hi_ = std::max(pos_hi_, dp.plen[s] + acc[s]);
      min_P_ = std::min(min_P_, dp.plen[s] + acc[s]);
    }
    draft_stats_[0] += 1;
    draft_stats_.push_back(total_P);
    have_prefill = true;
  }
  DevBuf draft_in;
  std::vector<int32_t> draft_stats_{0};

  void enqueue_step() {
    if (step.forks()) ensure_chain_streams(step.n_groups(B) - 1);
    step.enqueue_step();
  }
  void ensure_chain_streams(int n) {
    while ((int)chain_streams.size() < n) {
      hipStream_t s2;
      hipEvent_t e2;
      HIPCHK(hipStreamCreateWithFlags(&s2, hipStreamNonBlocking));
      HIPCHK(hipEventCreateWithFlags(&e2, hipEventDisableTiming));
      chain_streams.push_back(s2);
      join_ev.push_back(e2);
    }
    if (!fork_ev) HIPCHK(hipEventCreateWithFlags(&fork_ev, hipEventDisableTiming));
  }

  std::string make_graph_sig() const {
    uint64_t h = 1469598103934665603ull;
    DecodeStep::each_buf(step, [&](const DevBuf& sb) {
      uint64_t v = (uint64_t)(uintptr_t)sb.p;
      for (int i = 0; i < 8; ++i) { h ^= (v >> (8 * i)) & 0xff; h *= 1099511628211ull; }
    });
    char buf[256];
    snprintf(buf, sizeof(buf), "%d.%d.%d.%d.%d.%d.%d.%d.%d.%d.b%d.lb%d.sm%d.rp%d/%d/%d/%d/%p/%016llx", B, gsize, k_parallel_groups, k_skinny_q,
             k_dattn_batched_min_wgs, k_skinny_glu_hp3, k_lm_head_prune, (int)(min_P_ < 256), (int)head_logits_, (int)token_lp(), beam_w_, (int)logit_bias_on_, (int)sampling_on_, (int)repetition_on_, live_nsplit_,
             max_ctx, max_new, (const void*)arena, (unsigned long long)h);
    return buf;
  }

  template <class F> hipGraphExec_t capture_graph(F&& fn) {
    hipGraph_t g = nullptr;
    hipGraphExec_t exec = nullptr;
    HIPCHK(hipStreamBeginCapture(stream, hipStreamCaptureModeThreadLocal));
    try {
      fn();
    } catch (...) {
      hipGraph_t tmp = nullptr;
      (void)hipStreamEndCapture(stream, &tmp);
      if (tmp) (void)hipGraphDestroy(tmp);
      throw;
    }
    HIPCHK(hipStreamEndCapture(stream, &g));
    const hipError_t ie = hipGraphInstantiate(&exec, g, nullptr, nullptr, 0);
    (void)hipGraphDestroy(g);
    HIPCHK(ie);
    return exec;
  }
  hipGraphExec_t graph_for_step() {
    const std::string sig = make_graph_sig();
    for (size_t i = 0; i < graph_cache.size(); ++i)
      if (graph_cache[i].first == sig) {
        if (i + 1 != graph_cache.size()) std::rotate(graph_cache.begin() + i, graph_cache.begin() + i + 1, graph_cache.end());
        return graph_cache.back().second;
      }
    const hipGraphExec_t exec = capture_graph([&] { enqueue_step(); });
    ++graph_captures_;
    if (graph_cache.size() >= kGraphCacheMax) {
      retired_graphs.push_back(graph_cache.front().second);
      graph_cache.erase(graph_cache.begin());
    }
    graph_cache.emplace_back(sig, exec);
    return exec;
  }
  std::vector<hipGraphExec_t> retired_graphs;
  int32_t graph_captures_ = 0;
  void drain_retired_graphs() {
    for (auto ge : retired_graphs) (void)hipGraphExecDestroy(ge);
    retired_graphs.clear();
  }
  void drop_graphs() {
    drain_retired_graphs();
    for (auto& ge : graph_cache) (void)hipGraphExecDestroy(ge.second);
    graph_cache.clear();
  }

  void decode_steps(int n) {
    if (!have_prefill) fail("decode: no prefill state");
    if (n <= 0) return;
    const bool eager = !opts.use_graph || prof;
    const int kps = dattn_keys_per_split(kv_f32());
    for (int i = 0; i < n; ++i) {
      live_nsplit_ = step.uses_key_splits() ? std::min(attn_nsplit, pos_hi_ / kps + 1) : attn_nsplit;
      if (eager) enqueue_step();
      else HIPCHK(hipGraphLaunch(graph_for_step(), stream));
      ++pos_hi_;
    }
    if (eager) HIPCHK(hipGetLastError());
  }

  int max_new_request(int max_new_req, int fixed_new) const { return fixed_new > 0 ? fixed_new : max_new_req > 0 ? max_new_req : opts.max_new_tokens; }
  std::pair<std::vector<int32_t>, std::vector<int32_t>> asr_prompts(const int32_t* lang_ids, int n_prefix) const {
    return concat_prompts(B, [&](int s, int32_t* dst) {
      int32_t len = 0;
      q3a_build_prompt(T[s], lang_ids, n_prefix, dst, &len);
      return len;
    });
  }

  template <class Prompts>
  void whole_path_front(const char* what, const float* const* pcm16k, const int64_t* ns_in, int n, int width, int max_new_req, Prompts&& prompts) {
    if (!pcm16k || !ns_in || n < 1) fail(std::string(what) + ": bad argument");
    require_utterance_ptrs(what, pcm16k, n);
    HIPCHK(hipSetDevice(device));
    const int b = n * width;
    std::vector<const float*> ptrs((size_t)b);
    std::vector<int64_t> ns((size_t)b);
    for (int s = 0; s < b; ++s) { ptrs[s] = pcm16k[s / width]; ns[s] = ns_in[s / width]; }
    have_prefill = false;
    set_batch(ns.data(), b);
    auto&& [ids_v, lens_v] = prompts();
    setup_prompts(ids_v.data(), lens_v.data(), b, max_new_req, true);
    timings = q3a_timings{};
    upload_ptrs_and_mel(ptrs.data(), ns.data(), b);
    run_encoder();
  }

  void run_resident(int fixed_new, bool front_done = false) {
    if (B <= 0) fail("q3a_run_resident: no batch uploaded");
    if (!front_done) {
      HIPCHK(hipEventRecord(ev[0], stream));
      run_mel();
      HIPCHK(hipEventRecord(ev[1], stream));
      run_encoder();
    }
    HIPCHK(hipEventRecord(ev[2], stream));
    run_prefill();
    HIPCHK(hipEventRecord(ev[3], stream));
    int steps = 0;
    static const bool host_timing = [] { const char* e = getenv("Q3A_DEBUG_HOST_TIMING"); return e && atoi(e) != 0; }();
    const auto h0 = std::chrono::steady_clock::now();
    if (fixed_new > 0) {
      steps = fixed_new - 1;
      decode_steps(steps);
      if (host_timing) fprintf(stderr, "[q3a host timing] %d graph launches enqueued in %.1f us\n", steps,
                               std::chrono::duration<double, std::micro>(std::chrono::steady_clock::now() - h0).count());
    } else {
      steps = run_ahead(host_prog, max_new - 1, "greedy");
    }
    HIPCHK(hipEventRecord(ev[4], stream));
    HIPCHK(hipStreamSynchronize(stream));
    HIPCHK(hipGetLastError());
    decode_timings(steps);
  }

  void fetch_ids(int32_t* out, int stride, int32_t* out_lens) {
    if (!have_prefill || beam_w_ > 0) fail("q3a_fetch_ids: nothing generated");
    std::vector<int> all((size_t)B * max_new);
    HIPCHK(hipMemcpy(all.data(), step.out_ids.p, all.size() * 4, hipMemcpyDeviceToHost));
    generated_lens(all, out_lens);
    for (int s = 0; s < B; ++s)
      for (int i = 0; i < std::min(out_lens[s], stride); ++i) out[(size_t)s * stride + i] = all[(size_t)s * max_new + i];
  }
  void generated_lens(const std::vector<int>& all, int32_t* out_lens) {
    std::vector<int> sc(B);
    HIPCHK(hipMemcpy(sc.data(), step.step_count.p, (size_t)B * 4, hipMemcpyDeviceToHost));
    for (int s = 0; s < B; ++s) {
      int n = std::min(sc[s], max_new), len = 0;
      for (; len < n; ++len) {
        int t = all[(size_t)s * max_new + len];
        if (!fixed_mode_ && (t == kEos0 || t == kEos1)) break;
      }
      out_lens[s] = len;
    }
  }
  void fetch_logprobs(float* out, int stride, int32_t* out_lens) {
    if (!token_lp()) fail("q3a_fetch_logprobs: the engine was created without opts.token_logprobs = 1");
    if (!have_prefill) fail("q3a_fetch_logprobs: nothing generated");
    std::vector<int> all((size_t)B * max_new);
    std::vector<float> lp((size_t)B * max_new);
    HIPCHK(hipMemcpy(all.data(), step.out_ids.p, all.size() * 4, hipMemcpyDeviceToHost));
    HIPCHK(hipMemcpy(lp.data(), step.out_lp.p, lp.size() * 4, hipMemcpyDeviceToHost));
    generated_lens(all, out_lens);
    for (int s = 0; s < B; ++s)
      for (int i = 0; i < std::min(out_lens[s], stride); ++i) out[(size_t)s * stride + i] = lp[(size_t)s * max_new + i];
  }

  int beam_dbg_S_ = 0, beam_dbg_W_ = 0;
  int* beam_prog() const { return host_prog + 2; }

  void beam_check(const char* what, int W) const {
    if (W < 1 || W > BEAM_MAX_W) fail(std::string(what) + ": width must be 1..8");
    if (B % W != 0) fail(std::string(what) + ": the batch of " + std::to_string(B) + " sequences is not divisible by width " + std::to_string(W));
    if (B > 32) fail(std::string(what) + ": utterances x width = " + std::to_string(B) + " exceeds 32 sequences");
    for (int s = 0; s < B; ++s)
      if (P[s] != P[s / W * W]) fail(std::string(what) + ": the prompts of utterance " + std::to_string(s / W) + " differ in length (its " + std::to_string(W) + " slots must hold the same prompt)");
    if (d.vocab < W) fail(std::string(what) + ": vocabulary smaller than the width");
  }
  void set_logit_bias(const int32_t* ids, const float* bias, int n, float default_bias) {
    const char* what = "q3a_set_logit_bias";
    require_asr(what);
    const int V = d.vocab;
    if (n < 0 || (n > 0 && (!ids || !bias))) fail(std::string(what) + ": bad argument");
    if (!(default_bias == 0.f || default_bias == -INFINITY)) fail(std::string(what) + ": default_bias must be 0 or -inf");
    std::vector<float> b((size_t)V, default_bias);
    std::vector<uint8_t> seen((size_t)V, 0);
    for (int i = 0; i < n; ++i) {
      const int id = ids[i];
      if (id < 0 || id >= V) fail(std::string(what) + ": id " + std::to_string(id) + " is outside the vocabulary (" + std::to_string(V) + ")");
      if (seen[id]) fail(std::string(what) + ": duplicate id " + std::to_string(id));
      seen[id] = 1;
      const float v = bias[i];
      if (std::isnan(v) || v == INFINITY) fail(std::string(what) + ": the bias of id " + std::to_string(id) + " is NaN or +inf (finite or -inf only)");
      b[id] = v;
    }
    int finite = 0;
    for (int r = 0; r < V; ++r) finite += b[r] != -INFINITY;
    if (finite == 0) fail(std::string(what) + ": the bias has no finite entry (every token would be suppressed)");
    const bool on = !(n == 0 && default_bias == 0.f);
    const bool eos_open = (kEos0 < V && b[kEos0] != -INFINITY) || (kEos1 < V && b[kEos1] != -INFINITY);
    repetition_bias_check(what, rep_ngram_, eos_open, finite);
    have_prefill = false; beam_w_ = 0;
    HIPCHK(hipMemcpyAsync(step.logit_bias.p, b.data(), (size_t)V * 4, hipMemcpyHostToDevice, stream));
    HIPCHK(hipStreamSynchronize(stream));
    logit_bias_on_ = on;
    logit_bias_finite_ = finite;
    logit_bias_eos_open_ = eos_open;
  }
  void set_repetition(float penalty, int ngram) {
    const char* what = "q3a_set_repetition";
    require_asr(what);
    if (!std::isfinite(penalty) || !(penalty > 0.f)) fail(std::string(what) + ": repetition_penalty must be finite and > 0 (1 turns the penalty off)");
    if (ngram < 0 || ngram > 32) fail(std::string(what) + ": no_repeat_ngram_size must lie in [0, 32] (0 turns the ban off)");
    const bool on = !(penalty == 1.f && ngram == 0);
    if (on && d.vocab > REPEAT_MAX_VOCAB)
      fail(std::string(what) + ": the vocabulary (" + std::to_string(d.vocab) + ") exceeds the " + std::to_string(REPEAT_MAX_VOCAB) + " ids the kernel's bitmap holds");
    repetition_bias_check(what, ngram, logit_bias_eos_open_, logit_bias_finite_);
    uint32_t w[4] = {0, (uint32_t)ngram, 0, 0};
    memcpy(&w[0], &penalty, 4);
    have_prefill = false; beam_w_ = 0;
    HIPCHK(hipMemcpyAsync(step.rep_params.p, w, 16, hipMemcpyHostToDevice, stream));
    HIPCHK(hipStreamSynchronize(stream));
    rep_penalty_ = penalty; rep_ngram_ = ngram;
    repetition_on_ = on;
  }
  void repetition_bias_check(const char* what, int ngram, bool eos_open, int finite) const {
    if (ngram > 0 && !eos_open && finite <= opts.max_new_tokens)
      fail(std::string(what) + ": no_repeat_ngram_size " + std::to_string(ngram) + " over a logit bias that forbids both EOS ids and leaves " + std::to_string(finite) +
           " tokens finite, no more than max_new_tokens (" + std::to_string(opts.max_new_tokens) + "): a row could run out of finite logits");
  }
  void beam_repetition_check(const char* what) const {
    if (repetition_on_) fail(std::string(what) + ": repetition control is on (q3a_set_repetition); beam slots reorder their histories -- turn it off first");
  }
  void set_sampling(float temperature, float min_p, uint64_t seed) {
    const char* what = "q3a_set_sampling";
    require_asr(what);
    if (!(temperature >= 0.f) || !std::isfinite(temperature)) fail(std::string(what) + ": temperature must be finite and >= 0 (0 turns sampling off)");
    if (!(min_p >= 0.f && min_p <= 1.f)) fail(std::string(what) + ": min_p must lie in [0, 1]");
    uint32_t w[4];
    memcpy(&w[0], &temperature, 4); memcpy(&w[1], &min_p, 4);
    w[2] = (uint32_t)seed; w[3] = (uint32_t)(seed >> 32);
    have_prefill = false; beam_w_ = 0;
    HIPCHK(hipMemcpyAsync(step.samp_params.p, w, 16, hipMemcpyHostToDevice, stream));
    HIPCHK(hipStreamSynchronize(stream));
    memcpy(samp_words_, w, 16);
    sampling_on_ = temperature > 0.f;
  }
  void beam_sampling_check(const char* what) const {
    if (sampling_on_) fail(std::string(what) + ": sampling is on (q3a_set_sampling with temperature > 0); beam search selects deterministically -- turn it off first");
  }
  void beam_bias_check(const char* what, int W) const {
    if (logit_bias_on_ && W > logit_bias_finite_)
      fail(std::string(what) + ": width " + std::to_string(W) + " exceeds the " + std::to_string(logit_bias_finite_) + " tokens the logit bias leaves finite");
  }

  void beam_begin(const char* what, int W) {
    if (!have_prefill) fail(std::string(what) + ": no prefill state (call q3a_prefill first)");
    beam_check(what, W);
    beam_sampling_check(what);
    beam_repetition_check(what);
    beam_bias_check(what, W);
    if (!head_logits_ || pos_hi_ != *std::max_element(P.begin(), P.end()))
      fail(std::string(what) + ": needs the logits of q3a_prefill (call it directly after the prefill)");
    const int S = B, nc = beam_topk_chunks(d.vocab);
    step.beam_cand_val.ensure((size_t)S * nc * W * 4); step.beam_cand_idx.ensure((size_t)S * nc * W * 4);
    step.beam_part_max.ensure((size_t)S * nc * 4); step.beam_part_sum.ensure((size_t)S * nc * 4);
    step.beam_topk_ids.ensure((size_t)S * W * 4); step.beam_topk_lp.ensure((size_t)S * W * 4);
    step.beam_parent.ensure((size_t)S * 4); step.beam_token.ensure((size_t)S * 4); step.beam_feed.ensure((size_t)S * 4);
    step.beam_hist_parent.ensure((size_t)max_new * S * 4); step.beam_hist_token.ensure((size_t)max_new * S * 4); step.beam_hist_lp.ensure((size_t)max_new * S * 4);
    std::vector<float> sc((size_t)S, -INFINITY);
    for (int s = 0; s < S; s += W) sc[s] = 0.f;
    std::vector<uint8_t> fin((size_t)S, 0);
    std::vector<int> st(BEAM_ST_COUNT, 0);
    upload(step.beam_score, sc, stream); upload(step.beam_finished, fin, stream); upload(step.beam_state, st, stream); upload(step.beam_lo, P, stream);
    HIPCHK(hipStreamSynchronize(stream));
    __atomic_store_n(&beam_prog()[0], 0, __ATOMIC_RELAXED);
    __atomic_store_n(&beam_prog()[1], 0, __ATOMIC_RELAXED);
    beam_w_ = W; beam_dbg_S_ = S; beam_dbg_W_ = W;
    step.enqueue_beam_round();
    HIPCHK(hipGetLastError());
  }
  int run_ahead(const int* prog, int limit, const char* label, int base = 0) {
    const int ahead = std::max(1, knobs().eos_run_ahead.load());
    int steps = 0;
    unsigned spins = 0;
    while (steps < limit) {
      if (__atomic_load_n(&prog[1], __ATOMIC_RELAXED)) break;
      const int fin = __atomic_load_n(&prog[0], __ATOMIC_RELAXED);
      if (steps - std::max(fin - 1 - base, 0) < ahead) {
        decode_steps(1);
        ++steps;
        spins = 0;
      } else if (++spins > 64) {
        sched_yield();
        if ((spins & 0xffff) == 0) {
          const hipError_t q = hipStreamQuery(stream);
          if (q != hipSuccess && q != hipErrorNotReady) HIPCHK(q);
          if (q == hipSuccess && steps - std::max(__atomic_load_n(&prog[0], __ATOMIC_RELAXED) - 1 - base, 0) >= ahead)
            fail(std::string(label) + " loop: the stream drained but the device-side progress counter did not advance");
        }
      }
    }
    return steps;
  }
  std::vector<int> beam_state_host() {
    std::vector<int> st(BEAM_ST_COUNT);
    HIPCHK(hipStreamSynchronize(stream));
    HIPCHK(hipMemcpy(st.data(), step.beam_state.p, st.size() * 4, hipMemcpyDeviceToHost));
    return st;
  }
  void beam_fetch(int32_t* out, int stride, int32_t* out_lens, float* out_scores, uint8_t* out_fin, float* out_lp) {
    if (beam_w_ <= 0) fail("q3a_beam_fetch: no beam search (call q3a_beam_begin first)");
    const int W = beam_w_, S = B, U = B / W;
    const int R = std::min(beam_state_host()[BEAM_ST_ROUNDS], max_new);
    std::vector<int> hp((size_t)R * S), ht((size_t)R * S);
    std::vector<float> hl((size_t)R * S), sc(S);
    std::vector<uint8_t> fin(S);
    if (R > 0) {
      HIPCHK(hipMemcpy(hp.data(), step.beam_hist_parent.p, hp.size() * 4, hipMemcpyDeviceToHost));
      HIPCHK(hipMemcpy(ht.data(), step.beam_hist_token.p, ht.size() * 4, hipMemcpyDeviceToHost));
      HIPCHK(hipMemcpy(hl.data(), step.beam_hist_lp.p, hl.size() * 4, hipMemcpyDeviceToHost));
    }
    HIPCHK(hipMemcpy(sc.data(), step.beam_score.p, (size_t)S * 4, hipMemcpyDeviceToHost));
    HIPCHK(hipMemcpy(fin.data(), step.beam_finished.p, (size_t)S, hipMemcpyDeviceToHost));
    std::vector<int> toks;
    std::vector<float> lps;
    for (int u = 0; u < U; ++u) {
      std::vector<int> order(W);
      for (int j = 0; j < W; ++j) order[j] = j;
      std::stable_sort(order.begin(), order.end(), [&](int x, int y) { return sc[u * W + x] > sc[u * W + y]; });
      for (int k = 0; k < W; ++k) {
        const int q = u * W + order[k];
        toks.clear(); lps.clear();
        for (int r = R - 1, cur = q; r >= 0; --r) {
          const size_t h = (size_t)r * S + cur;
          if (ht[h] >= 0) { toks.push_back(ht[h]); lps.push_back(hl[h]); }
          cur = hp[h];
        }
        std::reverse(toks.begin(), toks.end());
        std::reverse(lps.begin(), lps.end());
        const int n_lp = (int)toks.size();
        if (fin[q] && !toks.empty()) toks.pop_back();
        const int n = (int)toks.size();
        if (n > stride) fail("q3a_beam_fetch: a hypothesis has " + std::to_string(n) + " ids, more than stride " + std::to_string(stride));
        const size_t o = (size_t)u * W + k;
        for (int i = 0; i < n; ++i) out[o * stride + i] = toks[i];
        out_lens[o] = n;
        if (out_scores) out_scores[o] = sc[q];
        if (out_fin) out_fin[o] = fin[q];
        if (out_lp)
          for (int i = 0; i < n_lp && i < stride + 1; ++i) out_lp[o * (stride + 1) + i] = lps[i];
      }
    }
  }

  ~q3a_engine() {
    drop_graphs();
    for (auto cs : chain_streams) (void)hipStreamDestroy(cs);
    for (auto ce : join_ev) (void)hipEventDestroy(ce);
    if (fork_ev) (void)hipEventDestroy(fork_ev);
    if (own_arena && arena) (void)hipFree(arena);
    if (host_prog) (void)hipHostFree(host_prog);
    if (up_stream) { (void)hipStreamSynchronize(up_stream); (void)hipStreamDestroy(up_stream); }
    if (pin_p) (void)hipHostFree(pin_p);
    for (auto ue : up_ev) (void)hipEventDestroy(ue);
    if (up_t0) (void)hipEventDestroy(up_t0);
    if (up_t1) (void)hipEventDestroy(up_t1);
    for (auto& x : ev)
      if (x) (void)hipEventDestroy(x);
    if (stream) (void)hipStreamDestroy(stream);
  }
};


namespace q3a {
void set_thread_error(const std::string& msg) { g_last_error = msg; }
void set_error(q3a_engine* e, const char* msg) {
  if (e) e->err = msg;
  g_last_error = msg;
}
}

extern "C" {

void q3a_opts_default(q3a_opts* o) {
  memset(o, 0, sizeof(*o));
  o->precise = 0;
  o->max_new_tokens = 4096;
  o->use_graph = 1;
  o->debug_taps = 0;
}

static int32_t create_impl(const char* model_dir, int32_t device, void* dev_arena, uint64_t bytes, const q3a_opts* opts,
                           q3a_engine** out) {
  q3a_engine* e = nullptr;
  try {
    if (!model_dir || !out) fail("null argument");
    e = new q3a_engine();
    e->init_common(model_dir, device, opts);
    if (dev_arena) {
      if (bytes != e->L.total) fail("q3a_engine_create_from_arena: arena size does not match config.json");
      e->arena = (uint8_t*)dev_arena;
      e->own_arena = false;
    } else {
      Checkpoint ck(model_dir);
      std::vector<uint8_t> host(e->L.total);
      pack_arena(e->d, e->L, ck, host.data());
      HIPCHK(hipMalloc((void**)&e->arena, e->L.total));
      e->own_arena = true;
      HIPCHK(hipMemcpy(e->arena, host.data(), e->L.total, hipMemcpyHostToDevice));
    }
    e->check_arena_header();
    e->init_tables();
    e->init_lm_head_q();
    *out = e;
    return 0;
  } catch (const std::exception& ex) {
    g_last_error = ex.what();
    delete e;
    if (out) *out = nullptr;
    return 1;
  }
}

int32_t q3a_device_count(void) {
  int n = 0;
  return hipGetDeviceCount(&n) == hipSuccess ? n : 0;
}

int32_t q3a_engine_create(const char* model_dir, int32_t device, const q3a_opts* opts, q3a_engine** out) {
  return create_impl(model_dir, device, nullptr, 0, opts, out);
}
int32_t q3a_engine_create_from_arena(const char* model_dir, int32_t device, void* device_arena, uint64_t bytes,
                                     const q3a_opts* opts, q3a_engine** out) {
  if (!device_arena) { g_last_error = "null arena"; return 1; }
  return create_impl(model_dir, device, device_arena, bytes, opts, out);
}

int32_t q3a_arena_bytes(const char* model_dir, uint64_t* bytes) {
  q3a_engine* e = nullptr;
  Q3A_TRY(e)
  Dims d = parse_config_file(std::string(model_dir) + "/config.json");
  validate_dims(d);
  *bytes = plan_arena(d).total;
  Q3A_CATCH(e)
}
int32_t q3a_arena_pack(const char* model_dir, void* host_dst, uint64_t bytes) {
  q3a_engine* e = nullptr;
  Q3A_TRY(e)
  Dims d = parse_config_file(std::string(model_dir) + "/config.json");
  validate_dims(d);
  ArenaLayout L = plan_arena(d);
  if (bytes != L.total) fail("q3a_arena_pack: buffer size does not match q3a_arena_bytes");
  Checkpoint ck(model_dir);
  pack_arena(d, L, ck, (uint8_t*)host_dst);
  Q3A_CATCH(e)
}

void q3a_engine_destroy(q3a_engine* e) { delete e; }
const char* q3a_last_error(const q3a_engine* e) { return e ? e->err.c_str() : g_last_error.c_str(); }

int32_t q3a_get_dims(const q3a_engine* e, q3a_dims* o) {
  if (!e || !o) return 1;
  const Dims& d = e->d;
  memset(o, 0, sizeof(*o));
  o->enc_d_model = d.enc_d; o->enc_layers = d.enc_layers; o->enc_heads = d.enc_heads; o->enc_ffn = d.enc_ffn;
  o->num_mel_bins = d.n_mels; o->n_window = d.n_window; o->n_window_infer = d.n_window_infer; o->conv_channels = d.conv_ch;
  o->enc_output_dim = d.enc_out; o->max_source_positions = d.max_source_positions;
  o->vocab_size = d.vocab; o->hidden_size = d.hidden; o->intermediate_size = d.inter; o->dec_layers = d.dec_layers;
  o->num_q_heads = d.n_q; o->num_kv_heads = d.n_kv; o->head_dim = d.head_dim; o->tie_word_embeddings = d.tie_embeddings;
  o->mrope_interleaved = d.mrope_interleaved;
  for (size_t i = 0; i < 4 && i < d.mrope_section.size(); ++i) o->mrope_section[i] = d.mrope_section[i];
  o->rms_norm_eps = d.rms_eps; o->rope_theta = d.rope_theta;
  return 0;
}

int32_t q3a_weights_rounded(const q3a_engine* e) { return e && (e->arena_flags & kFlagWeightsRounded) ? 1 : 0; }

int64_t q3a_num_frames(int64_t n_samples) { return (n_samples + 159) / 160; }
int32_t q3a_num_audio_tokens(const q3a_engine* e, int64_t n_frames) { return e ? e->d.audio_tokens(n_frames) : -1; }

int32_t q3a_build_prompt(int32_t num_audio_tokens, const int32_t* lang_prefix_ids, int32_t n_prefix, int32_t* ids,
                         int32_t* len) {
  static const int32_t head[9] = {151644, 8948, 198, 151645, 198, 151644, 872, 198, 151669};
  static const int32_t tail[6] = {151670, 151645, 198, 151644, 77091, 198};
  if (!lang_prefix_ids) n_prefix = 0;
  int32_t n = 9 + num_audio_tokens + 6 + n_prefix;
  if (len) *len = n;
  if (!ids) return 0;
  int32_t* p = ids;
  for (int i = 0; i < 9; ++i) *p++ = head[i];
  for (int i = 0; i < num_audio_tokens; ++i) *p++ = kAudioPad;
  for (int i = 0; i < 6; ++i) *p++ = tail[i];
  for (int i = 0; i < n_prefix; ++i) *p++ = lang_prefix_ids[i];
  return 0;
}

int32_t q3a_aligner_info(const q3a_engine* e, int32_t* classify_num, int32_t* timestamp_token_id, float* segment_ms) {
  if (!e) return 1;
  if (classify_num) *classify_num = e->d.classify_num;
  if (timestamp_token_id) *timestamp_token_id = e->d.aligner() ? e->d.timestamp_token_id : 0;
  if (segment_ms) *segment_ms = e->d.aligner() ? e->d.timestamp_segment_ms : 0.f;
  return 0;
}

int32_t q3a_align(q3a_engine* e, const int32_t* ids, const int32_t* lens, int32_t B, int32_t* out_classes, int32_t stride,
                  int32_t* out_counts, float* logits_out) {
  if (!e) return 1;
  Q3A_TRY(e)
  e->require_aligner("q3a_align");
  if (!ids || !lens || B < 1 || !out_counts || stride < 0 || (stride > 0 && !out_classes)) fail("q3a_align: bad argument");
  HIPCHK(hipSetDevice(e->device));
  if (!e->have_enc) fail("q3a_align: no encoder output (call q3a_encode first)");
  if (B != e->B) fail("q3a_align: batch size differs from the encoded batch");
  const std::vector<int> rows = e->align_marker_rows(ids, lens, B, stride, out_counts);
  e->setup_prompts(ids, lens, B, 1);
  e->timings = q3a_timings{};
  e->run_align(rows, out_counts, stride, out_classes, logits_out);
  Q3A_CATCH(e)
}

int32_t q3a_align_batch_ptrs(q3a_engine* e, const float* const* pcm16k, const int64_t* n_samples, int32_t B, const int32_t* text_ids,
                             const int32_t* text_lens, int32_t* out_classes, int32_t stride, int32_t* out_counts) {
  if (!e) return 1;
  Q3A_TRY(e)
  e->require_aligner("q3a_align_batch");
  if (!text_lens || !out_counts || stride < 0 || (stride > 0 && !out_classes)) fail("q3a_align_batch: bad argument");
  std::vector<int> rows;
  e->whole_path_front("q3a_align_batch", pcm16k, n_samples, B, 1, 1, [&] {
    std::vector<int64_t> toff(B, 0);
    for (int s = 0; s < B; ++s) {
      if (text_lens[s] < 0 || (text_lens[s] > 0 && !text_ids)) fail("q3a_align_batch: bad text");
      if (s + 1 < B) toff[s + 1] = toff[s] + text_lens[s];
    }
    auto pr = concat_prompts(B, [&](int s, int32_t* dst) {
      int32_t len = 0;
      q3a_build_align_prompt(e->T[s], text_ids ? text_ids + toff[s] : nullptr, text_lens[s], dst, &len);
      return len;
    });
    rows = e->align_marker_rows(pr.first.data(), pr.second.data(), B, stride, out_counts);
    return pr;
  });
  e->run_align(rows, out_counts, stride, out_classes, nullptr);
  e->front_and_total_timings();
  Q3A_CATCH(e)
}

int32_t q3a_score(q3a_engine* e, const int32_t* prompt_ids, const int32_t* prompt_lens, const int32_t* target_ids,
                  const int32_t* target_lens, int32_t B, float* out_lp, int32_t* out_top_ids, float* out_top_lp, int32_t stride,
                  float* logits_out) {
  if (!e) return 1;
  Q3A_TRY(e)
  e->require_asr("q3a_score");
  if (!prompt_ids || !prompt_lens || !target_lens || B < 1 || stride < 0 || (stride > 0 && !out_lp)) fail("q3a_score: bad argument");
  HIPCHK(hipSetDevice(e->device));
  if (!e->have_enc) fail("q3a_score: no encoder output (call q3a_encode first)");
  if (B != e->B) fail("q3a_score: batch size differs from the encoded batch");
  const auto sp = e->score_plan("q3a_score", prompt_ids, prompt_lens, target_ids, target_lens, B, stride);
  e->have_prefill = false;
  e->setup_prompts(sp.ids.data(), sp.lens.data(), B, 1);
  e->timings = q3a_timings{};
  e->run_score(sp, target_lens, stride, out_lp, out_top_ids, out_top_lp, logits_out);
  Q3A_CATCH(e)
}

int32_t q3a_score_batch_ptrs(q3a_engine* e, const float* const* pcm16k, const int64_t* n_samples, int32_t B,
                             const int32_t* lang_prefix_ids, int32_t n_prefix, const int32_t* target_ids, const int32_t* target_lens,
                             float* out_lp, int32_t* out_top_ids, float* out_top_lp, int32_t stride) {
  if (!e) return 1;
  Q3A_TRY(e)
  e->require_asr("q3a_score_batch");
  if (!target_lens || stride < 0 || (stride > 0 && !out_lp) || n_prefix < 0) fail("q3a_score_batch: bad argument");
  q3a_engine::ScorePlan sp;
  e->whole_path_front("q3a_score_batch", pcm16k, n_samples, B, 1, 1, [&] {
    const auto pr = e->asr_prompts(lang_prefix_ids, n_prefix);
    sp = e->score_plan("q3a_score_batch", pr.first.data(), pr.second.data(), target_ids, target_lens, B, stride);
    return std::tie(sp.ids, sp.lens);
  });
  e->run_score(sp, target_lens, stride, out_lp, out_top_ids, out_top_lp, nullptr);
  e->front_and_total_timings();
  Q3A_CATCH(e)
}

int32_t q3a_beam_begin(q3a_engine* e, int32_t width) {
  if (!e) return 1;
  Q3A_TRY(e)
  e->require_asr("q3a_beam_begin");
  HIPCHK(hipSetDevice(e->device));
  e->beam_begin("q3a_beam_begin", width);
  HIPCHK(hipStreamSynchronize(e->stream));
  HIPCHK(hipGetLastError());
  Q3A_CATCH(e)
}

int32_t q3a_beam_step(q3a_engine* e, uint8_t* all_finished, float* logits_out) {
  if (!e) return 1;
  Q3A_TRY(e)
  e->require_asr("q3a_beam_step");
  HIPCHK(hipSetDevice(e->device));
  if (e->beam_w_ <= 0 || !e->have_prefill) fail("q3a_beam_step: no beam search (call q3a_beam_begin first)");
  if (e->beam_state_host()[BEAM_ST_ROUNDS] >= e->max_new) fail("q3a_beam_step: the round limit (max_new_tokens) is reached");
  e->head_logits_ = true;
  e->decode_steps(1);
  const std::vector<int> st = e->beam_state_host();
  HIPCHK(hipGetLastError());
  if (all_finished) *all_finished = st[BEAM_ST_ALL_DONE] ? 1 : 0;
  if (logits_out) HIPCHK(hipMemcpy(logits_out, e->step.logits.p, (size_t)e->B * e->d.vocab * 4, hipMemcpyDeviceToHost));
  Q3A_CATCH(e)
}

int32_t q3a_beam_fetch(q3a_engine* e, int32_t* out_ids, int32_t stride, int32_t* out_lens, float* out_scores, uint8_t* out_finished,
                       float* out_lp) {
  if (!e) return 1;
  Q3A_TRY(e)
  e->require_asr("q3a_beam_fetch");
  if (e->beam_w_ <= 0) fail("q3a_beam_fetch: no beam search (call q3a_beam_begin first)");
  if (!out_lens || stride < 0 || (stride > 0 && !out_ids)) fail("q3a_beam_fetch: bad argument");
  HIPCHK(hipSetDevice(e->device));
  e->beam_fetch(out_ids, stride, out_lens, out_scores, out_finished, out_lp);
  Q3A_CATCH(e)
}

int32_t q3a_beam_search_batch_ptrs(q3a_engine* e, const float* const* pcm16k, const int64_t* n_samples, int32_t U,
                                   const int32_t* lang_prefix_ids, int32_t n_prefix, int32_t width, int32_t max_new, int32_t* out_ids,
                                   int32_t stride, int32_t* out_lens, float* out_scores, uint8_t* out_finished, float* out_lp) {
  if (!e) return 1;
  Q3A_TRY(e)
  e->require_asr("q3a_beam_search_batch");
  if (U < 1 || !out_lens || stride < 0 || (stride > 0 && !out_ids) || n_prefix < 0) fail("q3a_beam_search_batch: bad argument");
  if (width < 1 || width > BEAM_MAX_W) fail("q3a_beam_search_batch: width must be 1..8");
  if ((int64_t)U * width > 32) fail("q3a_beam_search_batch: utterances x width = " + std::to_string((int64_t)U * width) + " exceeds 32 sequences");
  const int cap = e->opts.max_new_tokens, want = max_new <= 0 ? cap : std::min(max_new, cap);
  if (stride < want) fail("q3a_beam_search_batch: stride " + std::to_string(stride) + " is below max_new " + std::to_string(want));
  e->beam_sampling_check("q3a_beam_search_batch");
  e->beam_repetition_check("q3a_beam_search_batch");
  e->beam_bias_check("q3a_beam_search_batch", width);
  e->fixed_mode_ = false;
  e->head_logits_ = true;
  e->whole_path_front("q3a_beam_search_batch", pcm16k, n_samples, U, width, want, [&] { return e->asr_prompts(lang_prefix_ids, n_prefix); });
  HIPCHK(hipEventRecord(e->ev[2], e->stream));
  e->run_prefill();
  HIPCHK(hipEventRecord(e->ev[3], e->stream));
  e->beam_begin("q3a_beam_search_batch", width);
  e->run_ahead(e->beam_prog(), e->max_new - 1, "beam");
  HIPCHK(hipEventRecord(e->ev[4], e->stream));
  const std::vector<int> st = e->beam_state_host();
  HIPCHK(hipGetLastError());
  e->decode_timings(std::max(st[BEAM_ST_ROUNDS] - 1, 0));
  e->beam_fetch(out_ids, stride, out_lens, out_scores, out_finished, out_lp);
  e->beam_w_ = 0; e->have_prefill = false;
  Q3A_CATCH(e)
}

int32_t q3a_set_logit_bias(q3a_engine* e, const int32_t* ids, const float* bias, int32_t n, float default_bias) {
  if (!e) return 1;
  Q3A_TRY(e)
  HIPCHK(hipSetDevice(e->device));
  e->set_logit_bias(ids, bias, n, default_bias);
  Q3A_CATCH(e)
}

int32_t q3a_set_sampling(q3a_engine* e, float temperature, float min_p, uint64_t seed) {
  if (!e) return 1;
  Q3A_TRY(e)
  HIPCHK(hipSetDevice(e->device));
  e->set_sampling(temperature, min_p, seed);
  Q3A_CATCH(e)
}

int32_t q3a_set_repetition(q3a_engine* e, float repetition_penalty, int32_t no_repeat_ngram_size) {
  if (!e) return 1;
  Q3A_TRY(e)
  HIPCHK(hipSetDevice(e->device));
  e->set_repetition(repetition_penalty, no_repeat_ngram_size);
  Q3A_CATCH(e)
}

int32_t q3a_upload_pcm(q3a_engine* e, const float* pcm16k, const int64_t* n_samples, int32_t B) {
  if (!e) return 1;
  Q3A_TRY(e)
  HIPCHK(hipSetDevice(e->device));
  e->upload_pcm(pcm16k, n_samples, B);
  Q3A_CATCH(e)
}

int32_t q3a_mel(q3a_engine* e, const float* pcm16k, const int64_t* n_samples, int32_t B, float* mel_out,
                int32_t* n_frames_out) {
  if (!e) return 1;
  Q3A_TRY(e)
  HIPCHK(hipSetDevice(e->device));
  e->upload_pcm(pcm16k, n_samples, B);
  e->run_mel();
  HIPCHK(hipStreamSynchronize(e->stream));
  HIPCHK(hipGetLastError());
  if (n_frames_out)
    for (int u = 0; u < B; ++u) n_frames_out[u] = e->n_frames[u];
  if (mel_out) {
    size_t total = 0;
    for (int u = 0; u < B; ++u) total += (size_t)e->n_frames[u] * e->d.n_mels;
    HIPCHK(hipMemcpy(mel_out, e->mel.p, total * 4, hipMemcpyDeviceToHost));
  }
  Q3A_CATCH(e)
}

int32_t q3a_encode(q3a_engine* e, float* audio_embeds_out, int32_t* T_out) {
  if (!e) return 1;
  Q3A_TRY(e)
  HIPCHK(hipSetDevice(e->device));
  e->run_encoder();
  HIPCHK(hipStreamSynchronize(e->stream));
  HIPCHK(hipGetLastError());
  if (T_out)
    for (int u = 0; u < e->B; ++u) T_out[u] = e->T[u];
  if (audio_embeds_out)
    HIPCHK(hipMemcpy(audio_embeds_out, e->audio_embeds.p, (size_t)e->total_T * e->d.enc_out * 4, hipMemcpyDeviceToHost));
  Q3A_CATCH(e)
}

int32_t q3a_prefill(q3a_engine* e, const int32_t* ids, const int32_t* lens, int32_t B, float* last_logits_out,
                    int32_t* next_ids) {
  if (!e) return 1;
  Q3A_TRY(e)
  e->require_asr("q3a_prefill");
  HIPCHK(hipSetDevice(e->device));
  e->fixed_mode_ = false;
  e->head_logits_ = true;
  e->setup_prompts(ids, lens, B, e->opts.max_new_tokens);
  e->run_prefill();
  HIPCHK(hipStreamSynchronize(e->stream));
  HIPCHK(hipGetLastError());
  if (last_logits_out) HIPCHK(hipMemcpy(last_logits_out, e->step.logits.p, (size_t)B * e->d.vocab * 4, hipMemcpyDeviceToHost));
  if (next_ids) HIPCHK(hipMemcpy(next_ids, e->step.next_tok.p, (size_t)B * 4, hipMemcpyDeviceToHost));
  Q3A_CATCH(e)
}

int32_t q3a_decode_step(q3a_engine* e, int32_t* next_ids, uint8_t* done, float* logits_out) {
  if (!e) return 1;
  Q3A_TRY(e)
  e->require_asr("q3a_decode_step");
  if (e->beam_w_ > 0) fail("q3a_decode_step: a beam search owns the decode state (q3a_beam_step; a new q3a_prefill returns to the greedy step)");
  HIPCHK(hipSetDevice(e->device));
  {
    std::vector<int> pos(e->B);
    HIPCHK(hipMemcpy(pos.data(), e->step.d_pos.p, (size_t)e->B * 4, hipMemcpyDeviceToHost));
    for (int s = 0; s < e->B; ++s)
      if (pos[s] + 1 > e->max_ctx) fail("q3a_decode_step: KV cache capacity exhausted (max_new_tokens reached)");
  }
  e->head_logits_ = true;
  e->decode_steps(1);
  HIPCHK(hipStreamSynchronize(e->stream));
  HIPCHK(hipGetLastError());
  if (next_ids) HIPCHK(hipMemcpy(next_ids, e->step.next_tok.p, (size_t)e->B * 4, hipMemcpyDeviceToHost));
  if (done) HIPCHK(hipMemcpy(done, e->step.done.p, (size_t)e->B, hipMemcpyDeviceToHost));
  if (logits_out) HIPCHK(hipMemcpy(logits_out, e->step.logits.p, (size_t)e->B * e->d.vocab * 4, hipMemcpyDeviceToHost));
  Q3A_CATCH(e)
}

int32_t q3a_set_next_tokens(q3a_engine* e, const int32_t* ids, int32_t B) {
  if (!e) return 1;
  Q3A_TRY(e)
  HIPCHK(hipSetDevice(e->device));
  if (!e->have_prefill || B != e->B || e->beam_w_ > 0) fail("q3a_set_next_tokens: no decode state / batch mismatch");
  for (int s = 0; s < B; ++s)
    if (ids[s] < 0 || ids[s] >= e->d.vocab) fail("q3a_set_next_tokens: token id out of range");
  e->step.enqueue_forced_tokens(ids);
  HIPCHK(hipStreamSynchronize(e->stream));
  Q3A_CATCH(e)
}

int32_t q3a_run_resident(q3a_engine* e, const int32_t* lang_prefix_ids, int32_t n_prefix, int32_t max_new,
                         int32_t fixed_new_tokens) {
  if (!e) return 1;
  Q3A_TRY(e)
  e->require_asr("q3a_run_resident");
  HIPCHK(hipSetDevice(e->device));
  e->fixed_mode_ = fixed_new_tokens > 0;
  e->head_logits_ = e->opts.debug_taps != 0;
  e->have_mel = e->have_enc = e->have_prefill = false;
  if (e->B <= 0) fail("q3a_run_resident: no batch uploaded");
  const auto pr = e->asr_prompts(lang_prefix_ids, n_prefix);
  e->setup_prompts(pr.first.data(), pr.second.data(), e->B, e->max_new_request(max_new, fixed_new_tokens), true);
  e->run_resident(fixed_new_tokens);
  Q3A_CATCH(e)
}

int32_t q3a_fetch_ids(q3a_engine* e, int32_t* out_ids, int32_t stride, int32_t* out_lens) {
  if (!e) return 1;
  Q3A_TRY(e)
  HIPCHK(hipSetDevice(e->device));
  e->fetch_ids(out_ids, stride, out_lens);
  Q3A_CATCH(e)
}

int32_t q3a_fetch_logprobs(q3a_engine* e, float* out_lp, int32_t stride, int32_t* out_lens) {
  if (!e) return 1;
  Q3A_TRY(e)
  if (!out_lens || (stride > 0 && !out_lp)) fail("q3a_fetch_logprobs: bad argument");
  HIPCHK(hipSetDevice(e->device));
  e->fetch_logprobs(out_lp, stride, out_lens);
  Q3A_CATCH(e)
}

int32_t q3a_transcribe_batch_ptrs(q3a_engine* e, const float* const* pcm16k, const int64_t* n_samples, int32_t B,
                                  const int32_t* lang_prefix_ids, int32_t n_prefix, int32_t max_new, int32_t fixed_new_tokens,
                                  int32_t* out_ids, int32_t stride, int32_t* out_lens) {
  if (!e) return 1;
  Q3A_TRY(e)
  e->require_asr("q3a_transcribe_batch");
  const auto w0 = std::chrono::steady_clock::now();
  e->fixed_mode_ = fixed_new_tokens > 0;
  e->head_logits_ = e->opts.debug_taps != 0;
  e->whole_path_front("q3a_transcribe_batch", pcm16k, n_samples, B, 1, e->max_new_request(max_new, fixed_new_tokens),
                      [&] { return e->asr_prompts(lang_prefix_ids, n_prefix); });
  e->run_resident(fixed_new_tokens, true);
  e->fetch_ids(out_ids, stride, out_lens);
  if (e->io.mode != 0) {
    float ms = 0.f;
    if (hipEventSynchronize(e->up_t1) != hipSuccess || hipEventElapsedTime(&ms, e->up_t0, e->up_t1) != hipSuccess) { (void)hipGetLastError(); ms = 0.f; }
    e->io.h2d_ms = ms;
  }
  e->io.wall_ms = std::chrono::duration<float, std::milli>(std::chrono::steady_clock::now() - w0).count();
  Q3A_CATCH(e)
}

int32_t q3a_transcribe_batch(q3a_engine* e, const float* pcm16k, const int64_t* n_samples, int32_t B,
                             const int32_t* lang_prefix_ids, int32_t n_prefix, int32_t max_new, int32_t fixed_new_tokens,
                             int32_t* out_ids, int32_t stride, int32_t* out_lens) {
  if (!e) return 1;
  if (!pcm16k || !n_samples || B < 1) { e->err = "q3a_transcribe_batch: bad argument"; return 1; }
  std::vector<const float*> ptrs((size_t)B);
  int64_t off = 0;
  for (int u = 0; u < B; ++u) { ptrs[u] = pcm16k + off; off += n_samples[u]; }
  return q3a_transcribe_batch_ptrs(e, ptrs.data(), n_samples, B, lang_prefix_ids, n_prefix, max_new, fixed_new_tokens, out_ids, stride, out_lens);
}

int32_t q3a_prefill_draft(q3a_engine* e, const int32_t* prompt_ids, const int32_t* prompt_lens, const int32_t* draft_ids, const int32_t* draft_lens,
                          int32_t B, int32_t* accepted_out, int32_t* next_ids_out, float* logits_out) {
  if (!e) return 1;
  Q3A_TRY(e)
  const char* what = "q3a_prefill_draft";
  e->draft_check(what);
  if (!prompt_ids || !prompt_lens || !draft_lens || B < 1) fail(std::string(what) + ": bad argument");
  HIPCHK(hipSetDevice(e->device));
  if (!e->have_enc) fail(std::string(what) + ": no encoder output (call q3a_encode first)");
  if (B != e->B) fail(std::string(what) + ": batch size differs from the encoded batch");
  const auto dp = e->draft_plan(what, prompt_ids, prompt_lens, draft_ids, draft_lens, B, e->opts.max_new_tokens);
  e->fixed_mode_ = false;
  e->head_logits_ = true;
  e->have_prefill = false;
  e->setup_prompts(dp.ids.data(), dp.lens.data(), B, e->opts.max_new_tokens);
  e->timings = q3a_timings{};
  e->draft_stats_.assign(1, 0);
  std::vector<int> acc;
  e->run_prefill_draft(dp, acc, logits_out);
  for (int s = 0; s < B; ++s) {
    if (accepted_out) accepted_out[s] = acc[s];
    if (next_ids_out) next_ids_out[s] = acc[(size_t)B + s];
  }
  Q3A_CATCH(e)
}

int32_t q3a_transcribe_draft_batch_ptrs(q3a_engine* e, const float* const* pcm16k, const int64_t* n_samples, int32_t B,
                                        const int32_t* lang_prefix_ids, int32_t n_prefix, const int32_t* draft_ids, const int32_t* draft_lens,
                                        int32_t max_new, int32_t max_rounds, int32_t min_tail, int32_t* out_ids, int32_t stride,
                                        int32_t* out_lens, int32_t* accepted_out) {
  if (!e) return 1;
  Q3A_TRY(e)
  const char* what = "q3a_transcribe_draft_batch";
  e->draft_check(what);
  if (!draft_lens || !out_lens || stride < 0 || (stride > 0 && !out_ids) || n_prefix < 0 || B < 1) fail(std::string(what) + ": bad argument");
  const auto w0 = std::chrono::steady_clock::now();
  e->fixed_mode_ = false;
  e->head_logits_ = e->opts.debug_taps != 0;
  const int mn = e->max_new_request(max_new, 0), mn_eff = std::min(std::max(mn, 1), e->opts.max_new_tokens);
  std::pair<std::vector<int32_t>, std::vector<int32_t>> pr;
  q3a_engine::DraftPlan dp;
  e->whole_path_front(what, pcm16k, n_samples, B, 1, mn, [&] {
    pr = e->asr_prompts(lang_prefix_ids, n_prefix);
    dp = e->draft_plan(what, pr.first.data(), pr.second.data(), draft_ids, draft_lens, B, mn_eff);
    return std::tie(dp.ids, dp.lens);
  });
  e->draft_stats_.assign(1, 0);
  HIPCHK(hipEventRecord(e->ev[2], e->stream));
  std::vector<int> acc;
  std::vector<int32_t> cur, cur_lens(B), nxt;
  {
    size_t total = 0;
    for (int s = 0; s < B; ++s) { cur_lens[s] = draft_lens[s]; total += draft_lens[s]; }
    if (total) cur.assign(draft_ids, draft_ids + total);
  }
  for (int round = 0;; ++round) {
    e->run_prefill_draft(dp, acc, nullptr);
    int tail = 0;
    for (int s = 0; s < B; ++s) tail = std::max(tail, cur_lens[s] - acc[s] - 1);
    if (round + 1 >= max_rounds || tail < std::max(min_tail, 1)) break;
    nxt.clear();
    size_t off = 0;
    for (int s = 0; s < B; ++s) {
      int32_t need = 0;
      const size_t o = nxt.size();
      nxt.resize(o + (size_t)cur_lens[s] + 1);
      if (q3a_draft_next_round(cur.data() + off, cur_lens[s], acc[s], acc[(size_t)B + s], nxt.data() + o, cur_lens[s] + 1, &need) != 0)
        fail(std::string(what) + ": " + q3a_last_error(nullptr));
      off += cur_lens[s];
      cur_lens[s] = std::min(need, mn_eff);
      nxt.resize(o + cur_lens[s]);
    }
    cur.swap(nxt);
    dp = e->draft_plan(what, pr.first.data(), pr.second.data(), cur.data(), cur_lens.data(), B, mn_eff);
    e->setup_prompts(dp.ids.data(), dp.lens.data(), B, mn);
  }
  HIPCHK(hipEventRecord(e->ev[3], e->stream));
  int min_k = e->max_new;
  for (int s = 0; s < B; ++s) min_k = std::min(min_k, acc[s]);
  const int steps = e->run_ahead(e->host_prog, e->max_new - 1 - min_k, "draft", acc[0]);
  HIPCHK(hipEventRecord(e->ev[4], e->stream));
  HIPCHK(hipStreamSynchronize(e->stream));
  HIPCHK(hipGetLastError());
  e->decode_timings(steps);
  e->fetch_ids(out_ids, stride, out_lens);
  if (accepted_out)
    for (int s = 0; s < B; ++s) accepted_out[s] = acc[s];
  e->io.wall_ms = std::chrono::duration<float, std::milli>(std::chrono::steady_clock::now() - w0).count();
  Q3A_CATCH(e)
}

int32_t q3a_io_timings_last(const q3a_engine* e, q3a_io_timings* out) {
  if (!e || !out) return 1;
  *out = e->io;
  return 0;
}

int32_t q3a_stage_timings(const q3a_engine* e, q3a_timings* out) {
  if (!e || !out) return 1;
  *out = e->timings;
  return 0;
}

int32_t q3a_profile_decode_step(q3a_engine* e, q3a_kernel_profile* out) {
  if (!e || !out) return 1;
  Q3A_TRY(e)
  HIPCHK(hipSetDevice(e->device));
  if (!e->have_prefill) fail("q3a_profile_decode_step: no decode state");
  std::vector<ProfEvent> evs;
  e->prof = &evs;
  try {
    e->decode_steps(1);
    HIPCHK(hipStreamSynchronize(e->stream));
  } catch (...) {
    e->prof = nullptr;
    throw;
  }
  e->prof = nullptr;
  memset(out, 0, sizeof(*out));
  for (auto& pe : evs) {
    float ms = 0.f;
    HIPCHK(hipEventElapsedTime(&ms, pe.a, pe.b));
    out->total_us[pe.kclass] += ms * 1000.f;
    out->launches[pe.kclass] += 1;
    out->weight_bytes[pe.kclass] += pe.bytes;
    (void)hipEventDestroy(pe.a);
    (void)hipEventDestroy(pe.b);
  }
  Q3A_CATCH(e)
}

int32_t q3a_profile_weight_stream(q3a_engine* e, int32_t reps, float* avg_us, double* bytes_per_launch, int32_t* launches) {
  if (!e) return 1;
  Q3A_TRY(e)
  HIPCHK(hipSetDevice(e->device));
  if (!e->have_prefill) fail("q3a_profile_weight_stream: no decode state");
  if (e->B > kGemvMaxSeq) fail("q3a_profile_weight_stream: the GEMV path serves at most 2 sequences");
  if (reps < 1) reps = 1;
  const Dims& d = e->d;
  const int S = e->B;
  auto sweep = [&]() {
    for (int li = 0; li < d.dec_layers; ++li) {
      const DecLayerOff& l = e->L.dec[li];
      const auto pj = e->step.layer_projs(li);
      GemvArgs g = e->step.gemv_args(pj.qkv);
      g.x = e->step.x_dec.as<float>(); g.rms_w = e->wf(l.in_ln); g.out = e->step.s_qkv.as<float>();
      KCHK(launch_gemv(g, S, e->stream));
      GemvArgs u = e->step.gemv_args(pj.gu);
      u.x = e->step.x_dec.as<float>(); u.rms_w = e->wf(l.post_ln); u.out = e->step.s_act.as<float>();
      KCHK(launch_gemv(u, S, e->stream));
    }
  };
  const hipGraphExec_t ge = e->capture_graph([&] { for (int r = 0; r < reps; ++r) sweep(); });
  HIPCHK(hipGraphLaunch(ge, e->stream));
  HIPCHK(hipStreamSynchronize(e->stream));
  hipEvent_t a, b;
  HIPCHK(hipEventCreate(&a));
  HIPCHK(hipEventCreate(&b));
  float ms = 0.f;
  constexpr int kReplays = 3;
  for (int rep = 0; rep < kReplays; ++rep) {
    HIPCHK(hipEventRecord(a, e->stream));
    HIPCHK(hipGraphLaunch(ge, e->stream));
    HIPCHK(hipEventRecord(b, e->stream));
    HIPCHK(hipStreamSynchronize(e->stream));
    float t = 0.f;
    HIPCHK(hipEventElapsedTime(&t, a, b));
    ms += t / kReplays;
  }
  HIPCHK(hipGetLastError());
  (void)hipEventDestroy(a);
  (void)hipEventDestroy(b);
  (void)hipGraphExecDestroy(ge);
  const int n = reps * d.dec_layers * 2;
  if (avg_us) *avg_us = ms * 1000.f / (float)n;
  const auto pj0 = e->step.layer_projs(0);
  if (bytes_per_launch) *bytes_per_launch = (pj0.qkv.bytes + pj0.gu.bytes) / 2.0;
  if (launches) *launches = n;
  Q3A_CATCH(e)
}

int32_t q3a_debug_read(q3a_engine* e, const char* name, void* dst, uint64_t bytes, uint64_t* actual) {
  if (!e) return 1;
  Q3A_TRY(e)
  HIPCHK(hipSetDevice(e->device));
  auto give = [&](const void* src, size_t n, bool on_device) {
    if (actual) *actual = n;
    if (!dst) return;
    if (bytes < n) fail("q3a_debug_read: destination too small");
    if (!on_device) { memcpy(dst, src, n); return; }
    HIPCHK(hipStreamSynchronize(e->stream));
    HIPCHK(hipMemcpy(dst, src, n, hipMemcpyDeviceToHost));
  };
  const uint64_t device_bytes = g_device_bytes.load();
  const struct { const char* name; const void* src; size_t n; bool on_device; } scalars[] = {
      {"lm_head_prune_stats", e->step.prune_stats.p, 8, true},
      {"align_head_ms", &e->align_head_ms, 4, false},
      {"score_head_ms", &e->score_head_ms, 4, false},
      {"device_bytes", &device_bytes, 8, false},
      {"graph_captures", &e->graph_captures_, 4, false},
  };
  for (const auto& sc : scalars)
    if (strcmp(name, sc.name) == 0) { give(sc.src, sc.n, sc.on_device); return 0; }
  if (strcmp(name, "logit_bias") == 0) {
    e->require_asr("q3a_debug_read: logit_bias");
    give(e->step.logit_bias.p, (size_t)e->d.vocab * 4, true);
    return 0;
  }
  if (strcmp(name, "draft_stats") == 0) {
    give(e->draft_stats_.data(), e->draft_stats_.size() * 4, false);
    return 0;
  }
  if (strcmp(name, "sampling") == 0) {
    e->require_asr("q3a_debug_read: sampling");
    const uint32_t st[5] = {e->sampling_on_ ? 1u : 0u, e->samp_words_[0], e->samp_words_[1], e->samp_words_[2], e->samp_words_[3]};
    give(st, 20, false);
    return 0;
  }
  if (strcmp(name, "repetition") == 0) {
    e->require_asr("q3a_debug_read: repetition");
    uint32_t st[3] = {e->repetition_on_ ? 1u : 0u, 0u, (uint32_t)e->rep_ngram_};
    memcpy(&st[1], &e->rep_penalty_, 4);
    give(st, 12, false);
    return 0;
  }
  if (strcmp(name, "logit_bias_stats") == 0) {
    e->require_asr("q3a_debug_read: logit_bias");
    const int32_t st[2] = {e->logit_bias_on_ ? 1 : 0, e->logit_bias_finite_};
    give(st, 8, false);
    return 0;
  }
  const size_t bS = (size_t)e->beam_dbg_S_, bW = (size_t)e->beam_dbg_W_;
  const struct { const char* name; const DevBuf* buf; size_t n; } beams[] = {
      {"beam_topk_ids", &e->step.beam_topk_ids, bS * bW * 4}, {"beam_topk_lp", &e->step.beam_topk_lp, bS * bW * 4},
      {"beam_parent", &e->step.beam_parent, bS * 4}, {"beam_token", &e->step.beam_token, bS * 4}, {"beam_score", &e->step.beam_score, bS * 4},
      {"beam_finished", &e->step.beam_finished, bS}, {"beam_stats", &e->step.beam_state, 16},
  };
  for (const auto& bm : beams)
    if (strcmp(name, bm.name) == 0) {
      if (bS == 0) fail(std::string("q3a_debug_read: '") + name + "' before any beam search");
      give(bm.buf->p, bm.n, true);
      return 0;
    }
  auto it = e->taps.bufs.find(name);
  if (it == e->taps.bufs.end()) fail(std::string("q3a_debug_read: no tap named '") + name + "' (opts.debug_taps set?)");
  give(it->second.p, e->taps.bytes[name], true);
  Q3A_CATCH(e)
}

int32_t q3a_debug_set(const char* key, int32_t value) {
  if (!key) return 1;
  for (const KnobEntry& t : kKnobTable)
    if (strcmp(key, t.key) == 0) { (knobs().*t.field).store(value); return 0; }
  g_last_error = std::string("q3a_debug_set: unknown key '") + key + "'";
  return 1;
}

}
```

qwen3_asr_rs_amd/csrc/k_mel.hip:

```cpp
#include "dev.h"
#include "kernels.h"

namespace q3a {
namespace {

constexpr int N_FFT = 400, HOP = 160, N_FREQ = 201, DFT_COLS = 416, N_MELS = 128;
constexpr int FRAMES_PER_BLOCK = 32;
constexpr int SAMPLES_PER_BLOCK = (FRAMES_PER_BLOCK - 1) * HOP + N_FFT;
constexpr int P_STRIDE = 209;
constexpr int K_MEL = 202;

__device__ __forceinline__ unsigned float_key(float x) {
  unsigned u = __float_as_uint(x);
  return (u & 0x80000000u) ? ~u : (u | 0x80000000u);
}
__device__ __forceinline__ float key_float(unsigned k) {
  return __uint_as_float((k & 0x80000000u) ? (k & 0x7fffffffu) : ~k);
}

__global__ __launch_bounds__(256) void mel_kernel(MelBatch mb, const float* __restrict__ dft,
                                                  const float* __restrict__ filt_t) {
  __shared__ float s_lds[SAMPLES_PER_BLOCK + SAMPLES_PER_BLOCK / HOP + 8];
  __shared__ float p_lds[FRAMES_PER_BLOCK * P_STRIDE];
  const int b = blockIdx.y;
  const int F = mb.n_frames[b];
  const int f0 = blockIdx.x * FRAMES_PER_BLOCK;
  if (f0 >= F) return;
  const int64_t n = mb.n_samples[b];
  const int64_t Lp = (int64_t)F * HOP;
  const float* pcm = mb.pcm + mb.pcm_off[b];
  const int tid = threadIdx.x, lane = tid & 63, wave = tid >> 6, half = lane >> 5, l31 = lane & 31;

  for (int p = tid; p < SAMPLES_PER_BLOCK; p += 256) {
    int64_t i = (int64_t)f0 * HOP + p - N_FFT / 2;
    if (i < 0) i = -i;
    else if (i >= Lp) i = 2 * (Lp - 1) - i;
    float v = 0.f;
    if (i >= 0 && i < n) v = pcm[i];
    s_lds[p + p / HOP] = v;
  }
  for (int i = tid; i < FRAMES_PER_BLOCK * P_STRIDE; i += 256) p_lds[i] = 0.f;
  __syncthreads();

  const int a_base = l31 * (HOP + 1);
  for (int tile = wave; tile < DFT_COLS / 32; tile += 4) {
    f32x16_t acc;
#pragma unroll
    for (int r = 0; r < 16; ++r) acc[r] = 0.f;
    const float* bcol = dft + tile * 32 + l31;
#pragma unroll 4
    for (int nn = 0; nn < N_FFT; nn += 2) {
      const int m = nn + half;
      const float a = s_lds[a_base + m + (m >= HOP) + (m >= 2 * HOP)];
      const float bv = bcol[(size_t)m * DFT_COLS];
      acc = __builtin_amdgcn_mfma_f32_32x32x2f32(a, bv, acc, 0, 0, 0);
    }
    const int c = tile * 32 + l31, k = c >> 1;
#pragma unroll
    for (int r = 0; r < 16; ++r) {
      float pw = acc[r] * acc[r];
      pw += __shfl_xor(pw, 1, 64);
      const int frame = (r & 3) + 8 * (r >> 2) + 4 * half;
      if ((c & 1) == 0 && k < P_STRIDE - 1) p_lds[frame * P_STRIDE + k] = pw;
    }
  }
  __syncthreads();

  f32x16_t acc;
#pragma unroll
  for (int r = 0; r < 16; ++r) acc[r] = 0.f;
  const float* acol = filt_t + wave * 32 + l31;
  const float* brow = p_lds + l31 * P_STRIDE;
#pragma unroll 4
  for (int kk = 0; kk < K_MEL; kk += 2) {
    const int k = kk + half;
    acc = __builtin_amdgcn_mfma_f32_32x32x2f32(acol[(size_t)k * N_MELS], brow[k], acc, 0, 0, 0);
  }
  const int f = f0 + l31;
  float vmax = -3.0e38f;
  float* out = mb.mel + mb.mel_off[b];
#pragma unroll
  for (int r = 0; r < 16; ++r) {
    const int m = wave * 32 + (r & 3) + 8 * (r >> 2) + 4 * half;
    const float lv = log10f(fmaxf(acc[r], 1e-10f));
    if (f < F) {
      out[(size_t)m * F + f] = lv;
      vmax = fmaxf(vmax, lv);
    }
  }
  vmax = wave_max(vmax);
  if (lane == 0) atomicMax(mb.gmax_key + b, float_key(vmax));
}

__global__ void mel_finalize_kernel(MelBatch mb) {
  const int b = blockIdx.y;
  const int64_t total = (int64_t)mb.n_frames[b] * N_MELS;
  const float floor_v = key_float(mb.gmax_key[b]) - 8.0f;
  float* m = mb.mel + mb.mel_off[b];
  for (int64_t i = (int64_t)blockIdx.x * blockDim.x + threadIdx.x; i < total; i += (int64_t)gridDim.x * blockDim.x)
    m[i] = (fmaxf(m[i], floor_v) + 4.0f) / 4.0f;
}

}

const char* launch_mel(const MelBatch& mb, int B, int max_frames, const float* dft, const float* filt_t,
                       hipStream_t s) {
  if (B <= 0) return nullptr;
  hipError_t e = hipMemsetAsync(mb.gmax_key, 0, sizeof(unsigned) * B, s);
  if (e != hipSuccess) return "mel: memset failed";
  const int tiles = (max_frames + FRAMES_PER_BLOCK - 1) / FRAMES_PER_BLOCK;
  hipLaunchKernelGGL(mel_kernel, dim3(tiles, B), dim3(256), 0, s, mb, dft, filt_t);
  int fb = (max_frames * N_MELS + 255) / 256;
  if (fb > 1024) fb = 1024;
  hipLaunchKernelGGL(mel_finalize_kernel, dim3(fb, B), dim3(256), 0, s, mb);
  return nullptr;
}

}
```

Before: 491.2 audio-seconds/sec.

## Defer host syncs, stage uploads via pinned arena, prefetch mel MFMA operands

Several unrelated changes land together. Small host-to-device uploads now go through a pinned staging arena so the copies can be truly asynchronous. The sync inside prompt setup moves to a lazy begin_call/sync_done drain, and results come back through a pinned async readback fused into the final sync. Separately, the mel kernel's DFT and filterbank MFMA loops are rewritten to double-buffer global and LDS operand loads a block ahead with sched barriers, which adds register pressure.

Result: no change. 492.8 audio-seconds/sec, median of 2 (+0.3%).

```diff
diff --git a/qwen3_asr_rs_amd/csrc/engine.cpp b/qwen3_asr_rs_amd/csrc/engine.cpp
--- a/qwen3_asr_rs_amd/csrc/engine.cpp
+++ b/qwen3_asr_rs_amd/csrc/engine.cpp
@@ -21,10 +21,43 @@
 
 constexpr int kGemvMaxSeq = 2;
 
+struct PinArena {
+  struct Block { char* p; size_t cap; };
+  std::vector<Block> blocks;
+  size_t used = 0;
+  void* take(size_t bytes) {
+    bytes = (bytes + 63) & ~size_t(63);
+    if (blocks.empty() || used + bytes > blocks.back().cap) {
+      size_t total = 0;
+      for (const Block& b : blocks) total += b.cap;
+      const size_t want = (std::max(std::max(bytes, total), size_t(64) << 10) + 4095) & ~size_t(4095);
+      void* p = nullptr;
+      HIPCHK(hipHostMalloc(&p, want, hipHostMallocDefault));
+      blocks.push_back(Block{(char*)p, want});
+      used = 0;
+    }
+    void* r = blocks.back().p + used;
+    used += bytes;
+    return r;
+  }
+  void rewind() {
+    while (blocks.size() > 1) { (void)hipHostFree(blocks.front().p); blocks.erase(blocks.begin()); }
+    used = 0;
+  }
+  void release() {
+    for (const Block& b : blocks) (void)hipHostFree(b.p);
+    blocks.clear();
+    used = 0;
+  }
+};
+
 template <typename T>
-void upload(DevBuf& b, const std::vector<T>& v, hipStream_t s) {
+void upload(DevBuf& b, const std::vector<T>& v, PinArena& staging, hipStream_t s) {
   b.ensure(std::max<size_t>(v.size() * sizeof(T), 16));
-  if (!v.empty()) HIPCHK(hipMemcpyAsync(b.p, v.data(), v.size() * sizeof(T), hipMemcpyHostToDevice, s));
+  if (v.empty()) return;
+  void* h = staging.take(v.size() * sizeof(T));
+  memcpy(h, v.data(), v.size() * sizeof(T));
+  HIPCHK(hipMemcpyAsync(b.p, h, v.size() * sizeof(T), hipMemcpyHostToDevice, s));
 }
 
 struct ProfEvent {
@@ -579,6 +612,53 @@
 
   float stage_ms(int i, int j) { float ms = 0.f; HIPCHK(hipEventElapsedTime(&ms, ev[i], ev[j])); return ms; }
 
+  bool in_flight_ = false;
+  int32_t call_drains_ = 0;
+  PinArena staging_;
+  int32_t* res_pin_ = nullptr;
+  size_t res_cap_ = 0;
+  bool res_fresh_ = false;
+
+  void busy() { in_flight_ = true; }
+  template <typename T> void upload(DevBuf& b, const std::vector<T>& v, hipStream_t s) {
+    busy();
+    ::upload(b, v, staging_, s);
+  }
+  void sync_done() {
+    HIPCHK(hipStreamSynchronize(stream));
+    for (auto cs : chain_streams) HIPCHK(hipStreamSynchronize(cs));
+    in_flight_ = false;
+  }
+  void begin_call() {
+    if (in_flight_) {
+      ++call_drains_;
+      sync_done();
+    }
+    drain_retired_graphs();
+    staging_.rewind();
+  }
+  void reset_progress() {
+    __atomic_store_n(&host_prog[0], 0, __ATOMIC_RELAXED);
+    __atomic_store_n(&host_prog[1], 0, __ATOMIC_RELAXED);
+  }
+  void enqueue_results() {
+    const size_t n_ids = (size_t)B * max_new, words = n_ids + (size_t)B;
+    if (words > res_cap_) {
+      if (res_pin_) (void)hipHostFree(res_pin_);
+      res_pin_ = nullptr; res_cap_ = 0;
+      const size_t want = (words + 1023) & ~size_t(1023);
+      HIPCHK(hipHostMalloc((void**)&res_pin_, want * 4, hipHostMallocDefault));
+      res_cap_ = want;
+    }
+    HIPCHK(hipMemcpyAsync(res_pin_, step.out_ids.p, n_ids * 4, hipMemcpyDeviceToHost, stream));
+    HIPCHK(hipMemcpyAsync(res_pin_ + n_ids, step.step_count.p, (size_t)B * 4, hipMemcpyDeviceToHost, stream));
+  }
+  static bool host_timing() {
+    static const bool on = [] { const char* e = getenv("Q3A_DEBUG_HOST_TIMING"); return e && atoi(e) != 0; }();
+    return on;
+  }
+  std::chrono::steady_clock::time_point t_entry_;
+
   void init_common(const std::string& model_dir, int dev, const q3a_opts* o) {
     if (o) opts = *o; else q3a_opts_default(&opts);
     if (opts.max_new_tokens <= 0) opts.max_new_tokens = 4096;
@@ -621,7 +701,8 @@
     zero_page.ensure(256);
     HIPCHK(hipMemsetAsync(zero_page.p, 0, 256, stream));
     ensure_rope(8192);
-    HIPCHK(hipStreamSynchronize(stream));
+    sync_done();
+    staging_.release();
   }
 
   void ensure_rope(int n_pos) {
@@ -632,7 +713,7 @@
     HIPCHK(hipStreamSynchronize(stream));
     upload(step.rope_cos, c, stream);
     upload(step.rope_sin, s, stream);
-    HIPCHK(hipStreamSynchronize(stream));
+    sync_done();
     rope_positions = n;
   }
 
@@ -724,7 +805,7 @@
     upload(enc_segs, enc_segs_h, stream);
     mel.ensure((size_t)mo * 4);
     gmax.ensure((size_t)b * 4);
-    HIPCHK(hipStreamSynchronize(stream));
+    sync_done();
     B = b;
     geom_valid = true;
   }
@@ -733,10 +814,11 @@
     set_batch(ns, b);
     int64_t src = 0;
     for (int u = 0; u < b; ++u) {
+      busy();
       HIPCHK(hipMemcpyAsync(pcm.as<float>() + pcm_off[u], host + src, (size_t)ns[u] * 4, hipMemcpyHostToDevice, stream));
       src += ns[u];
     }
-    HIPCHK(hipStreamSynchronize(stream));
+    sync_done();
   }
 
   void upload_ptrs_and_mel(const float* const* ptrs, const int64_t* ns, int b) {
@@ -747,6 +829,9 @@
     static const int pieces_env = [] { const char* e = getenv("Q3A_UPLOAD_PIECES"); return e ? atoi(e) : 8; }();
     io = q3a_io_timings{};
     io.mode = mode;
+    busy();
+    if (host_timing()) fprintf(stderr, "[q3a host timing] entry -> first launch %.1f us\n",
+                               std::chrono::duration<double, std::micro>(std::chrono::steady_clock::now() - t_entry_).count());
     HIPCHK(hipEventRecord(ev[0], stream));
     const size_t total = (size_t)(pcm_off[b - 1] + ((ns[b - 1] + 3) & ~int64_t(3))) * 4;
     bool staged = mode != 0;
@@ -761,7 +846,7 @@
     if (!staged) {
       for (int u = 0; u < b; ++u)
         HIPCHK(hipMemcpyAsync(pcm.as<float>() + pcm_off[u], ptrs[u], (size_t)ns[u] * 4, hipMemcpyHostToDevice, stream));
-      HIPCHK(hipStreamSynchronize(stream));
+      sync_done();
       io.pieces = b;
       run_mel();
       HIPCHK(hipEventRecord(ev[1], stream));
@@ -836,6 +921,7 @@
   void run_mel() {
     MelBatch mb{pcm.as<float>(), d_pcm_off.as<int64_t>(), d_n_samples.as<int64_t>(), d_mel_off.as<int64_t>(),
                 d_n_frames.as<int>(), mel.as<float>(), gmax.as<unsigned>()};
+    busy();
     KCHK(launch_mel(mb, B, max_frames, dft.as<float>(), filt_t.as<float>(), stream));
     mel_done();
   }
@@ -848,6 +934,7 @@
 
   void run_encoder() {
     if (!have_mel) fail("q3a_encode: no mel (call q3a_mel first)");
+    busy();
     const int C = d.conv_ch, D = d.enc_d, Fn = d.enc_ffn;
     const int H1 = Dims::conv_len(d.n_mels), W1 = Dims::conv_len(d.chunk_frames());
     const int H2 = Dims::conv_len(H1), W2 = Dims::conv_len(W1);
@@ -951,31 +1038,33 @@
     have_enc = true;
   }
 
-  void setup_prompts(const int32_t* ids_h, const int32_t* lens, int b, int max_new_req, bool before_encoder = false) {
+  void prompts_now(const int32_t* ids_h, const int32_t* lens, int b, int max_new_req) {
+    begin_call();
+    setup_prompts(ids_h, lens, b, max_new_req, false);
+    reset_progress();
+    commit_prompts(ids_h);
+  }
+
+  void setup_prompts(const int32_t* ids_h, const int32_t* lens, int b, int max_new_req, bool before_encoder) {
     if (!have_enc && !before_encoder) fail("q3a_prefill: no encoder output (call q3a_encode first)");
     if (b != B) fail("q3a_prefill: batch size differs from the encoded batch");
     P.assign(lens, lens + b);
     beam_w_ = 0;
     seq_off.resize(b);
-    std::vector<int> rowseq, rowpos, amap((size_t)total_T, -1), last(b);
     int off = 0, maxP = 0;
     for (int s = 0; s < b; ++s) {
       seq_off[s] = off;
       int na = 0;
       for (int i = 0; i < P[s]; ++i) {
-        rowseq.push_back(s);
-        rowpos.push_back(i);
         int id = ids_h[off + i];
         if (id < 0 || id >= d.vocab) fail("q3a_prefill: token id out of range");
         if (id == kAudioPad) {
           if (na >= T[s]) fail("q3a_prefill: more <|audio_pad|> tokens than encoder tokens");
-          amap[(size_t)tok_off[s] + na] = off + i;
           ++na;
         }
       }
       if (na != T[s]) fail("q3a_prefill: number of <|audio_pad|> tokens does not match the encoder output length");
       if (P[s] <= 0) fail("q3a_prefill: empty prompt");
-      last[s] = off + P[s] - 1;
       off += P[s];
       maxP = std::max(maxP, P[s]);
     }
@@ -989,18 +1078,10 @@
       if (pad > 0) max_ctx += (pad + 127) / 128 * 128;
     }
     ensure_rope(max_ctx + 1);
-    std::vector<int> ids_v(ids_h, ids_h + total_P);
-    std::vector<AttnSeg> segs(b);
-    for (int s = 0; s < b; ++s)
-      segs[s] = AttnSeg{seq_off[s], P[s], (int64_t)s * d.n_kv * max_ctx * 128};
-    upload(ids, ids_v, stream);
-    upload(row_seq, rowseq, stream);
-    upload(row_pos, rowpos, stream);
-    upload(audio_rowmap, amap, stream);
-    upload(last_rows, last, stream);
-    upload(dec_segs, segs, stream);
-    upload(step.d_pos, P, stream);
     const size_t Pt = (size_t)total_P, H = d.hidden;
+    ids.ensure(std::max<size_t>(Pt * 4, 16)); row_seq.ensure(std::max<size_t>(Pt * 4, 16)); row_pos.ensure(std::max<size_t>(Pt * 4, 16));
+    audio_rowmap.ensure(std::max<size_t>((size_t)total_T * 4, 16)); last_rows.ensure(std::max<size_t>((size_t)b * 4, 16));
+    dec_segs.ensure(std::max<size_t>((size_t)b * sizeof(AttnSeg), 16)); step.d_pos.ensure(std::max<size_t>((size_t)b * 4, 16));
     dec_x.ensure(Pt * H * 4); dec_ln.ensure(Pt * H * act_elem()); dec_qkv.ensure(Pt * d.qkv_dim() * 4);
     dec_ctx.ensure(Pt * d.q_dim() * (valu_attn() ? 4 : act_elem())); dec_act.ensure(Pt * d.inter * act_elem());
     if (!valu_attn()) dec_q16.ensure(Pt * d.q_dim() * 2);
@@ -1037,27 +1118,47 @@
       const size_t n_stat = (size_t)b * d.n_q * attn_nsplit;
       step.attn_pm.ensure((n_stat + 8) * 4); step.attn_pl.ensure((n_stat + 8) * 4);
       step.attn_po.ensure(n_stat * 128 * 4);
-      if (knobs().poison_attn_partials.load() != 0) {
-        HIPCHK(hipMemsetAsync(step.attn_pm.p, 0xFF, step.attn_pm.cap, stream));
-        HIPCHK(hipMemsetAsync(step.attn_pl.p, 0xFF, step.attn_pl.cap, stream));
-        HIPCHK(hipMemsetAsync(step.attn_po.p, 0xFF, step.attn_po.cap, stream));
-      }
+    }
+    {
+      bool any = false;
+      DecodeStep::each_buf(step, [&](DevBuf& sb) { any = any || sb.grew; sb.grew = false; });
+      if (any) drop_graphs();
+    }
+  }
+
+  void commit_prompts(const int32_t* ids_h) {
+    const int b = B;
+    res_fresh_ = false;
+    std::vector<int> rowseq((size_t)total_P), rowpos((size_t)total_P), amap((size_t)total_T, -1), last(b);
+    std::vector<AttnSeg> segs(b);
+    for (int s = 0; s < b; ++s) {
+      const int off = seq_off[s];
+      for (int i = 0, na = 0; i < P[s]; ++i) {
+        rowseq[(size_t)off + i] = s;
+        rowpos[(size_t)off + i] = i;
+        if (ids_h[off + i] == kAudioPad) amap[(size_t)tok_off[s] + na++] = off + i;
+      }
+      last[s] = off + P[s] - 1;
+      segs[s] = AttnSeg{off, P[s], (int64_t)s * d.n_kv * max_ctx * 128};
+    }
+    std::vector<int> ids_v(ids_h, ids_h + total_P);
+    upload(ids, ids_v, stream);
+    upload(row_seq, rowseq, stream);
+    upload(row_pos, rowpos, stream);
+    upload(audio_rowmap, amap, stream);
+    upload(last_rows, last, stream);
+    upload(dec_segs, segs, stream);
+    upload(step.d_pos, P, stream);
+    if (knobs().poison_attn_partials.load() != 0) {
+      HIPCHK(hipMemsetAsync(step.attn_pm.p, 0xFF, step.attn_pm.cap, stream));
+      HIPCHK(hipMemsetAsync(step.attn_pl.p, 0xFF, step.attn_pl.cap, stream));
+      HIPCHK(hipMemsetAsync(step.attn_po.p, 0xFF, step.attn_po.cap, stream));
     }
     HIPCHK(hipMemsetAsync(step.step_count.p, 0, (size_t)b * 4, stream));
     HIPCHK(hipMemsetAsync(step.done.p, 0, (size_t)b, stream));
     HIPCHK(hipMemsetAsync(step.n_done.p, 0, 64, stream));
     HIPCHK(hipMemsetAsync(step.out_ids.p, 0, (size_t)b * max_new * 4, stream));
     if (token_lp()) HIPCHK(hipMemsetAsync(step.out_lp.p, 0, (size_t)b * max_new * 4, stream));
-    HIPCHK(hipStreamSynchronize(stream));
-    for (auto cs : chain_streams) HIPCHK(hipStreamSynchronize(cs));
-    __atomic_store_n(&host_prog[0], 0, __ATOMIC_RELAXED);
-    __atomic_store_n(&host_prog[1], 0, __ATOMIC_RELAXED);
-    drain_retired_graphs();
-    {
-      bool any = false;
-      DecodeStep::each_buf(step, [&](DevBuf& sb) { any = any || sb.grew; sb.grew = false; });
-      if (any) drop_graphs();
-    }
   }
 
   void run_prefill() {
@@ -1074,6 +1175,7 @@
   void run_prefill_layers() {
     const int H = d.hidden, I = d.inter, QD = d.q_dim(), QKV = d.qkv_dim();
     const bool sp = precise();
+    busy();
     KCHK(launch_embed(ids.as<int>(), total_P, wh(L.embed), H, kAudioPad, dec_x.as<float>(), stream));
     KCHK(launch_scatter_rows(audio_embeds.as<float>(), audio_rowmap.as<int>(), total_T, d.hidden, dec_x.as<float>(), stream));
     tap("dec_embed", dec_x.p, (size_t)total_P * H * 4);
@@ -1177,7 +1279,7 @@
       enqueue_head();
     }
     HIPCHK(hipEventRecord(ev[4], stream));
-    HIPCHK(hipStreamSynchronize(stream));
+    sync_done();
     HIPCHK(hipGetLastError());
     timings.prefill_ms = stage_ms(2, 4);
     head_ms = stage_ms(3, 4);
@@ -1347,7 +1449,7 @@
     da.draft_off = draft_in.as<int>(); da.prompt_len = da.draft_off + B + 1; da.draft = da.prompt_len + B;
     da.top_id = a.top_id; da.top_lp = a.top_lp;
     step.enqueue_draft_accept(da);
-    HIPCHK(hipStreamSynchronize(stream));
+    sync_done();
     HIPCHK(hipGetLastError());
     acc.resize((size_t)2 * B);
     HIPCHK(hipMemcpy(acc.data(), step.draft_accepted.p, acc.size() * 4, hipMemcpyDeviceToHost));
@@ -1443,6 +1545,8 @@
   void decode_steps(int n) {
     if (!have_prefill) fail("decode: no prefill state");
     if (n <= 0) return;
+    busy();
+    res_fresh_ = false;
     const bool eager = !opts.use_graph || prof;
     const int kps = dattn_keys_per_split(kv_f32());
     for (int i = 0; i < n; ++i) {
@@ -1465,6 +1569,7 @@
 
   template <class Prompts>
   void whole_path_front(const char* what, const float* const* pcm16k, const int64_t* ns_in, int n, int width, int max_new_req, Prompts&& prompts) {
+    t_entry_ = std::chrono::steady_clock::now();
     if (!pcm16k || !ns_in || n < 1) fail(std::string(what) + ": bad argument");
     require_utterance_ptrs(what, pcm16k, n);
     HIPCHK(hipSetDevice(device));
@@ -1473,53 +1578,79 @@
     std::vector<int64_t> ns((size_t)b);
     for (int s = 0; s < b; ++s) { ptrs[s] = pcm16k[s / width]; ns[s] = ns_in[s / width]; }
     have_prefill = false;
+    begin_call();
     set_batch(ns.data(), b);
     auto&& [ids_v, lens_v] = prompts();
     setup_prompts(ids_v.data(), lens_v.data(), b, max_new_req, true);
+    reset_progress();
     timings = q3a_timings{};
     upload_ptrs_and_mel(ptrs.data(), ns.data(), b);
     run_encoder();
-  }
-
-  void run_resident(int fixed_new, bool front_done = false) {
+    commit_prompts(ids_v.data());
+  }
+
+  void run_resident(int fixed_new, const int32_t* prompt_ids = nullptr) {
     if (B <= 0) fail("q3a_run_resident: no batch uploaded");
-    if (!front_done) {
+    if (prompt_ids) {
+      busy();
+      if (host_timing()) fprintf(stderr, "[q3a host timing] entry -> first launch %.1f us\n",
+                                 std::chrono::duration<double, std::micro>(std::chrono::steady_clock::now() - t_entry_).count());
       HIPCHK(hipEventRecord(ev[0], stream));
       run_mel();
       HIPCHK(hipEventRecord(ev[1], stream));
       run_encoder();
+      commit_prompts(prompt_ids);
     }
     HIPCHK(hipEventRecord(ev[2], stream));
     run_prefill();
     HIPCHK(hipEventRecord(ev[3], stream));
     int steps = 0;
-    static const bool host_timing = [] { const char* e = getenv("Q3A_DEBUG_HOST_TIMING"); return e && atoi(e) != 0; }();
     const auto h0 = std::chrono::steady_clock::now();
     if (fixed_new > 0) {
       steps = fixed_new - 1;
       decode_steps(steps);
-      if (host_timing) fprintf(stderr, "[q3a host timing] %d graph launches enqueued in %.1f us\n", steps,
-                               std::chrono::duration<double, std::micro>(std::chrono::steady_clock::now() - h0).count());
+      if (host_timing()) fprintf(stderr, "[q3a host timing] %d graph launches enqueued in %.1f us\n", steps,
+                                 std::chrono::duration<double, std::micro>(std::chrono::steady_clock::now() - h0).count());
     } else {
       steps = run_ahead(host_prog, max_new - 1, "greedy");
     }
     HIPCHK(hipEventRecord(ev[4], stream));
-    HIPCHK(hipStreamSynchronize(stream));
+    finish_loop();
+    const auto h1 = std::chrono::steady_clock::now();
+    decode_timings(steps);
+    if (host_timing()) fprintf(stderr, "[q3a host timing] final sync -> return %.1f us\n",
+                               std::chrono::duration<double, std::micro>(std::chrono::steady_clock::now() - h1).count());
+  }
+  void finish_loop() {
+    enqueue_results();
+    sync_done();
     HIPCHK(hipGetLastError());
-    decode_timings(steps);
-  }
-
+    res_fresh_ = true;
+  }
+
+  void read_results(std::vector<int>& all, std::vector<int>& sc) {
+    all.resize((size_t)B * max_new);
+    sc.resize(B);
+    if (res_fresh_) {
+      memcpy(all.data(), res_pin_, all.size() * 4);
+      memcpy(sc.data(), res_pin_ + all.size(), (size_t)B * 4);
+      return;
+    }
+    HIPCHK(hipMemcpy(all.data(), step.out_ids.p, all.size() * 4, hipMemcpyDeviceToHost));
+    HIPCHK(hipMemcpy(sc.data(), step.step_count.p, (size_t)B * 4, hipMemcpyDeviceToHost));
+  }
   void fetch_ids(int32_t* out, int stride, int32_t* out_lens) {
     if (!have_prefill || beam_w_ > 0) fail("q3a_fetch_ids: nothing generated");
-    std::vector<int> all((size_t)B * max_new);
-    HIPCHK(hipMemcpy(all.data(), step.out_ids.p, all.size() * 4, hipMemcpyDeviceToHost));
-    generated_lens(all, out_lens);
+    const auto h0 = std::chrono::steady_clock::now();
+    std::vector<int> all, sc;
+    read_results(all, sc);
+    generated_lens(all, sc, out_lens);
     for (int s = 0; s < B; ++s)
       for (int i = 0; i < std::min(out_lens[s], stride); ++i) out[(size_t)s * stride + i] = all[(size_t)s * max_new + i];
-  }
-  void generated_lens(const std::vector<int>& all, int32_t* out_lens) {
-    std::vector<int> sc(B);
-    HIPCHK(hipMemcpy(sc.data(), step.step_count.p, (size_t)B * 4, hipMemcpyDeviceToHost));
+    if (host_timing()) fprintf(stderr, "[q3a host timing] fetch_ids %.1f us (%s)\n",
+                               std::chrono::duration<double, std::micro>(std::chrono::steady_clock::now() - h0).count(), res_fresh_ ? "result block" : "copies");
+  }
+  void generated_lens(const std::vector<int>& all, const std::vector<int>& sc, int32_t* out_lens) {
     for (int s = 0; s < B; ++s) {
       int n = std::min(sc[s], max_new), len = 0;
       for (; len < n; ++len) {
@@ -1532,11 +1663,11 @@
   void fetch_logprobs(float* out, int stride, int32_t* out_lens) {
     if (!token_lp()) fail("q3a_fetch_logprobs: the engine was created without opts.token_logprobs = 1");
     if (!have_prefill) fail("q3a_fetch_logprobs: nothing generated");
-    std::vector<int> all((size_t)B * max_new);
+    std::vector<int> all, sc;
     std::vector<float> lp((size_t)B * max_new);
-    HIPCHK(hipMemcpy(all.data(), step.out_ids.p, all.size() * 4, hipMemcpyDeviceToHost));
+    read_results(all, sc);
     HIPCHK(hipMemcpy(lp.data(), step.out_lp.p, lp.size() * 4, hipMemcpyDeviceToHost));
-    generated_lens(all, out_lens);
+    generated_lens(all, sc, out_lens);
     for (int s = 0; s < B; ++s)
       for (int i = 0; i < std::min(out_lens[s], stride); ++i) out[(size_t)s * stride + i] = lp[(size_t)s * max_new + i];
   }
@@ -1577,7 +1708,7 @@
     repetition_bias_check(what, rep_ngram_, eos_open, finite);
     have_prefill = false; beam_w_ = 0;
     HIPCHK(hipMemcpyAsync(step.logit_bias.p, b.data(), (size_t)V * 4, hipMemcpyHostToDevice, stream));
-    HIPCHK(hipStreamSynchronize(stream));
+    sync_done();
     logit_bias_on_ = on;
     logit_bias_finite_ = finite;
     logit_bias_eos_open_ = eos_open;
@@ -1595,7 +1726,7 @@
     memcpy(&w[0], &penalty, 4);
     have_prefill = false; beam_w_ = 0;
     HIPCHK(hipMemcpyAsync(step.rep_params.p, w, 16, hipMemcpyHostToDevice, stream));
-    HIPCHK(hipStreamSynchronize(stream));
+    sync_done();
     rep_penalty_ = penalty; rep_ngram_ = ngram;
     repetition_on_ = on;
   }
@@ -1617,7 +1748,7 @@
     w[2] = (uint32_t)seed; w[3] = (uint32_t)(seed >> 32);
     have_prefill = false; beam_w_ = 0;
     HIPCHK(hipMemcpyAsync(step.samp_params.p, w, 16, hipMemcpyHostToDevice, stream));
-    HIPCHK(hipStreamSynchronize(stream));
+    sync_done();
     memcpy(samp_words_, w, 16);
     sampling_on_ = temperature > 0.f;
   }
@@ -1648,7 +1779,7 @@
     std::vector<uint8_t> fin((size_t)S, 0);
     std::vector<int> st(BEAM_ST_COUNT, 0);
     upload(step.beam_score, sc, stream); upload(step.beam_finished, fin, stream); upload(step.beam_state, st, stream); upload(step.beam_lo, P, stream);
-    HIPCHK(hipStreamSynchronize(stream));
+    sync_done();
     __atomic_store_n(&beam_prog()[0], 0, __ATOMIC_RELAXED);
     __atomic_store_n(&beam_prog()[1], 0, __ATOMIC_RELAXED);
     beam_w_ = W; beam_dbg_S_ = S; beam_dbg_W_ = W;
@@ -1680,7 +1811,7 @@
   }
   std::vector<int> beam_state_host() {
     std::vector<int> st(BEAM_ST_COUNT);
-    HIPCHK(hipStreamSynchronize(stream));
+    sync_done();
     HIPCHK(hipMemcpy(st.data(), step.beam_state.p, st.size() * 4, hipMemcpyDeviceToHost));
     return st;
   }
@@ -1736,6 +1867,8 @@
     if (fork_ev) (void)hipEventDestroy(fork_ev);
     if (own_arena && arena) (void)hipFree(arena);
     if (host_prog) (void)hipHostFree(host_prog);
+    staging_.release();
+    if (res_pin_) (void)hipHostFree(res_pin_);
     if (up_stream) { (void)hipStreamSynchronize(up_stream); (void)hipStreamDestroy(up_stream); }
     if (pin_p) (void)hipHostFree(pin_p);
     for (auto ue : up_ev) (void)hipEventDestroy(ue);
@@ -1889,7 +2022,7 @@
   if (!e->have_enc) fail("q3a_align: no encoder output (call q3a_encode first)");
   if (B != e->B) fail("q3a_align: batch size differs from the encoded batch");
   const std::vector<int> rows = e->align_marker_rows(ids, lens, B, stride, out_counts);
-  e->setup_prompts(ids, lens, B, 1);
+  e->prompts_now(ids, lens, B, 1);
   e->timings = q3a_timings{};
   e->run_align(rows, out_counts, stride, out_classes, logits_out);
   Q3A_CATCH(e)
@@ -1933,7 +2066,7 @@
   if (B != e->B) fail("q3a_score: batch size differs from the encoded batch");
   const auto sp = e->score_plan("q3a_score", prompt_ids, prompt_lens, target_ids, target_lens, B, stride);
   e->have_prefill = false;
-  e->setup_prompts(sp.ids.data(), sp.lens.data(), B, 1);
+  e->prompts_now(sp.ids.data(), sp.lens.data(), B, 1);
   e->timings = q3a_timings{};
   e->run_score(sp, target_lens, stride, out_lp, out_top_ids, out_top_lp, logits_out);
   Q3A_CATCH(e)
@@ -1963,7 +2096,7 @@
   e->require_asr("q3a_beam_begin");
   HIPCHK(hipSetDevice(e->device));
   e->beam_begin("q3a_beam_begin", width);
-  HIPCHK(hipStreamSynchronize(e->stream));
+  e->sync_done();
   HIPCHK(hipGetLastError());
   Q3A_CATCH(e)
 }
@@ -2066,7 +2199,7 @@
   HIPCHK(hipSetDevice(e->device));
   e->upload_pcm(pcm16k, n_samples, B);
   e->run_mel();
-  HIPCHK(hipStreamSynchronize(e->stream));
+  e->sync_done();
   HIPCHK(hipGetLastError());
   if (n_frames_out)
     for (int u = 0; u < B; ++u) n_frames_out[u] = e->n_frames[u];
@@ -2083,7 +2216,7 @@
   Q3A_TRY(e)
   HIPCHK(hipSetDevice(e->device));
   e->run_encoder();
-  HIPCHK(hipStreamSynchronize(e->stream));
+  e->sync_done();
   HIPCHK(hipGetLastError());
   if (T_out)
     for (int u = 0; u < e->B; ++u) T_out[u] = e->T[u];
@@ -2100,9 +2233,9 @@
   HIPCHK(hipSetDevice(e->device));
   e->fixed_mode_ = false;
   e->head_logits_ = true;
-  e->setup_prompts(ids, lens, B, e->opts.max_new_tokens);
+  e->prompts_now(ids, lens, B, e->opts.max_new_tokens);
   e->run_prefill();
-  HIPCHK(hipStreamSynchronize(e->stream));
+  e->sync_done();
   HIPCHK(hipGetLastError());
   if (last_logits_out) HIPCHK(hipMemcpy(last_logits_out, e->step.logits.p, (size_t)B * e->d.vocab * 4, hipMemcpyDeviceToHost));
   if (next_ids) HIPCHK(hipMemcpy(next_ids, e->step.next_tok.p, (size_t)B * 4, hipMemcpyDeviceToHost));
@@ -2123,7 +2256,7 @@
   }
   e->head_logits_ = true;
   e->decode_steps(1);
-  HIPCHK(hipStreamSynchronize(e->stream));
+  e->sync_done();
   HIPCHK(hipGetLastError());
   if (next_ids) HIPCHK(hipMemcpy(next_ids, e->step.next_tok.p, (size_t)e->B * 4, hipMemcpyDeviceToHost));
   if (done) HIPCHK(hipMemcpy(done, e->step.done.p, (size_t)e->B, hipMemcpyDeviceToHost));
@@ -2138,8 +2271,10 @@
   if (!e->have_prefill || B != e->B || e->beam_w_ > 0) fail("q3a_set_next_tokens: no decode state / batch mismatch");
   for (int s = 0; s < B; ++s)
     if (ids[s] < 0 || ids[s] >= e->d.vocab) fail("q3a_set_next_tokens: token id out of range");
+  e->busy();
+  e->res_fresh_ = false;
   e->step.enqueue_forced_tokens(ids);
-  HIPCHK(hipStreamSynchronize(e->stream));
+  e->sync_done();
   Q3A_CATCH(e)
 }
 
@@ -2148,14 +2283,17 @@
   if (!e) return 1;
   Q3A_TRY(e)
   e->require_asr("q3a_run_resident");
+  e->t_entry_ = std::chrono::steady_clock::now();
   HIPCHK(hipSetDevice(e->device));
   e->fixed_mode_ = fixed_new_tokens > 0;
   e->head_logits_ = e->opts.debug_taps != 0;
   e->have_mel = e->have_enc = e->have_prefill = false;
   if (e->B <= 0) fail("q3a_run_resident: no batch uploaded");
+  e->begin_call();
   const auto pr = e->asr_prompts(lang_prefix_ids, n_prefix);
   e->setup_prompts(pr.first.data(), pr.second.data(), e->B, e->max_new_request(max_new, fixed_new_tokens), true);
-  e->run_resident(fixed_new_tokens);
+  e->reset_progress();
+  e->run_resident(fixed_new_tokens, pr.first.data());
   Q3A_CATCH(e)
 }
 
@@ -2187,7 +2325,7 @@
   e->head_logits_ = e->opts.debug_taps != 0;
   e->whole_path_front("q3a_transcribe_batch", pcm16k, n_samples, B, 1, e->max_new_request(max_new, fixed_new_tokens),
                       [&] { return e->asr_prompts(lang_prefix_ids, n_prefix); });
-  e->run_resident(fixed_new_tokens, true);
+  e->run_resident(fixed_new_tokens);
   e->fetch_ids(out_ids, stride, out_lens);
   if (e->io.mode != 0) {
     float ms = 0.f;
@@ -2223,7 +2361,7 @@
   e->fixed_mode_ = false;
   e->head_logits_ = true;
   e->have_prefill = false;
-  e->setup_prompts(dp.ids.data(), dp.lens.data(), B, e->opts.max_new_tokens);
+  e->prompts_now(dp.ids.data(), dp.lens.data(), B, e->opts.max_new_tokens);
   e->timings = q3a_timings{};
   e->draft_stats_.assign(1, 0);
   std::vector<int> acc;
@@ -2283,15 +2421,14 @@
     }
     cur.swap(nxt);
     dp = e->draft_plan(what, pr.first.data(), pr.second.data(), cur.data(), cur_lens.data(), B, mn_eff);
-    e->setup_prompts(dp.ids.data(), dp.lens.data(), B, mn);
+    e->prompts_now(dp.ids.data(), dp.lens.data(), B, mn);
   }
   HIPCHK(hipEventRecord(e->ev[3], e->stream));
   int min_k = e->max_new;
   for (int s = 0; s < B; ++s) min_k = std::min(min_k, acc[s]);
   const int steps = e->run_ahead(e->host_prog, e->max_new - 1 - min_k, "draft", acc[0]);
   HIPCHK(hipEventRecord(e->ev[4], e->stream));
-  HIPCHK(hipStreamSynchronize(e->stream));
-  HIPCHK(hipGetLastError());
+  e->finish_loop();
   e->decode_timings(steps);
   e->fetch_ids(out_ids, stride, out_lens);
   if (accepted_out)
@@ -2321,7 +2458,7 @@
   e->prof = &evs;
   try {
     e->decode_steps(1);
-    HIPCHK(hipStreamSynchronize(e->stream));
+    e->sync_done();
   } catch (...) {
     e->prof = nullptr;
     throw;
@@ -2363,7 +2500,7 @@
   };
   const hipGraphExec_t ge = e->capture_graph([&] { for (int r = 0; r < reps; ++r) sweep(); });
   HIPCHK(hipGraphLaunch(ge, e->stream));
-  HIPCHK(hipStreamSynchronize(e->stream));
+  e->sync_done();
   hipEvent_t a, b;
   HIPCHK(hipEventCreate(&a));
   HIPCHK(hipEventCreate(&b));
@@ -2373,7 +2510,7 @@
     HIPCHK(hipEventRecord(a, e->stream));
     HIPCHK(hipGraphLaunch(ge, e->stream));
     HIPCHK(hipEventRecord(b, e->stream));
-    HIPCHK(hipStreamSynchronize(e->stream));
+    e->sync_done();
     float t = 0.f;
     HIPCHK(hipEventElapsedTime(&t, a, b));
     ms += t / kReplays;
@@ -2399,7 +2536,7 @@
     if (!dst) return;
     if (bytes < n) fail("q3a_debug_read: destination too small");
     if (!on_device) { memcpy(dst, src, n); return; }
-    HIPCHK(hipStreamSynchronize(e->stream));
+    e->sync_done();
     HIPCHK(hipMemcpy(dst, src, n, hipMemcpyDeviceToHost));
   };
   const uint64_t device_bytes = g_device_bytes.load();
@@ -2409,6 +2546,7 @@
       {"score_head_ms", &e->score_head_ms, 4, false},
       {"device_bytes", &device_bytes, 8, false},
       {"graph_captures", &e->graph_captures_, 4, false},
+      {"call_drains", &e->call_drains_, 4, false},
   };
   for (const auto& sc : scalars)
     if (strcmp(name, sc.name) == 0) { give(sc.src, sc.n, sc.on_device); return 0; }
diff --git a/qwen3_asr_rs_amd/csrc/k_mel.hip b/qwen3_asr_rs_amd/csrc/k_mel.hip
--- a/qwen3_asr_rs_amd/csrc/k_mel.hip
+++ b/qwen3_asr_rs_amd/csrc/k_mel.hip
@@ -16,6 +16,35 @@
 }
 __device__ __forceinline__ float key_float(unsigned k) {
   return __uint_as_float((k & 0x80000000u) ? (k & 0x7fffffffu) : ~k);
+}
+
+template <int N, int KB, bool GlobalIsA, class LoadG, class LoadL>
+__device__ __forceinline__ f32x16_t mfma_blocks_ahead(f32x16_t acc, LoadG lg, LoadL ll) {
+  constexpr int NB = (N + KB - 1) / KB;
+  float g[2][KB], l[2][KB];
+#pragma unroll
+  for (int i = 0; i < KB; ++i)
+    if (i < N) g[0][i] = lg(i);
+#pragma unroll
+  for (int i = 0; i < KB; ++i)
+    if (i < N) l[0][i] = ll(i);
+#pragma unroll
+  for (int blk = 0; blk < NB; ++blk) {
+    const int cur = blk & 1, nxt = cur ^ 1;
+#pragma unroll
+    for (int i = 0; i < KB; ++i)
+      if ((blk + 1) * KB + i < N) g[nxt][i] = lg((blk + 1) * KB + i);
+#pragma unroll
+    for (int i = 0; i < KB; ++i)
+      if ((blk + 1) * KB + i < N) l[nxt][i] = ll((blk + 1) * KB + i);
+    __builtin_amdgcn_sched_barrier(0);
+#pragma unroll
+    for (int i = 0; i < KB; ++i)
+      if (blk * KB + i < N)
+        acc = __builtin_amdgcn_mfma_f32_32x32x2f32(GlobalIsA ? g[cur][i] : l[cur][i], GlobalIsA ? l[cur][i] : g[cur][i], acc, 0, 0, 0);
+    __builtin_amdgcn_sched_barrier(0);
+  }
+  return acc;
 }
 
 __global__ __launch_bounds__(256) void mel_kernel(MelBatch mb, const float* __restrict__ dft,
@@ -48,13 +77,9 @@
 #pragma unroll
     for (int r = 0; r < 16; ++r) acc[r] = 0.f;
     const float* bcol = dft + tile * 32 + l31;
-#pragma unroll 4
-    for (int nn = 0; nn < N_FFT; nn += 2) {
-      const int m = nn + half;
-      const float a = s_lds[a_base + m + (m >= HOP) + (m >= 2 * HOP)];
-      const float bv = bcol[(size_t)m * DFT_COLS];
-      acc = __builtin_amdgcn_mfma_f32_32x32x2f32(a, bv, acc, 0, 0, 0);
-    }
+    acc = mfma_blocks_ahead<N_FFT / 2, 25, false>(
+        acc, [&](int j) { return bcol[(size_t)(2 * j + half) * DFT_COLS]; },
+        [&](int j) { return s_lds[a_base + 2 * j + half + (2 * j >= HOP) + (2 * j >= 2 * HOP)]; });
     const int c = tile * 32 + l31, k = c >> 1;
 #pragma unroll
     for (int r = 0; r < 16; ++r) {
@@ -71,11 +96,8 @@
   for (int r = 0; r < 16; ++r) acc[r] = 0.f;
   const float* acol = filt_t + wave * 32 + l31;
   const float* brow = p_lds + l31 * P_STRIDE;
-#pragma unroll 4
-  for (int kk = 0; kk < K_MEL; kk += 2) {
-    const int k = kk + half;
-    acc = __builtin_amdgcn_mfma_f32_32x32x2f32(acol[(size_t)k * N_MELS], brow[k], acc, 0, 0, 0);
-  }
+  acc = mfma_blocks_ahead<K_MEL / 2, 26, true>(
+      acc, [&](int j) { return acol[(size_t)(2 * j + half) * N_MELS]; }, [&](int j) { return brow[2 * j + half]; });
   const int f = f0 + l31;
   float vmax = -3.0e38f;
   float* out = mb.mel + mb.mel_off[b];
```
